# vstroebel/jpeg-encoder

Measured on NVIDIA B200. Metric: megapixels/sec encoded, byte-identical to the reference restatement, higher is better.
Workload: dtype u8 in / i32 arithmetic / i16 coefficients

## Files before the change

jpeg_encoder_b200/csrc/api.cu:

```cuda
#include <cuda_runtime.h>

#include <cstdio>
#include <cstdlib>
#include <algorithm>
#include <cstring>
#include <string>
#include <condition_variable>
#include <mutex>
#include <thread>
#include <vector>

#include "../../include/jpegenc_b200.h"
#include "copy_pool.h"
#include "host.h"
#include "kernels.h"

using namespace jpgb;

namespace {

bool poison_alloc() {
    const char *e = std::getenv("JPGB_POISON_ALLOC");
    return e && e[0] == '1';
}

struct DevBuf {
    void *p = nullptr;
    size_t cap = 0;
    cudaError_t reserve(size_t bytes) {
        if (bytes <= cap) return cudaSuccess;
        if (p) cudaFree(p);
        p = nullptr;
        cap = 0;
        size_t want = bytes + bytes / 8 + 256;
        want = (want + 255) & ~(size_t)255;
        cudaError_t e = cudaMalloc(&p, want);
        if (e == cudaSuccess) cap = want;
        if (e == cudaSuccess && poison_alloc()) {
            e = cudaMemset(p, 0xFF, want);
            if (e == cudaSuccess) e = cudaDeviceSynchronize();
        }
        return e;
    }
    template <typename T>
    T *as() const { return static_cast<T *>(p); }
    void release() {
        if (p) cudaFree(p);
        p = nullptr;
        cap = 0;
    }
};

struct PinnedBuf {
    void *p = nullptr;
    size_t cap = 0;
    cudaError_t reserve(size_t bytes) {
        if (bytes <= cap) return cudaSuccess;
        if (p) cudaFreeHost(p);
        p = nullptr;
        cap = 0;
        const size_t want = bytes + bytes / 8 + 256;
        cudaError_t e = cudaMallocHost(&p, want);
        if (e == cudaSuccess) {
            cap = want;
            if (poison_alloc()) std::memset(p, 0xFF, want);
        }
        return e;
    }
    template <typename T>
    T *as() const { return static_cast<T *>(p); }
    void release() {
        if (p) cudaFreeHost(p);
        p = nullptr;
        cap = 0;
    }
};

}

namespace {
struct PlanSig {
    jpgb_params p;
    jpgb_strip strip;
    uint32_t is_strip, planar;
};
inline PlanSig plan_sig(const Plan &plan) {
    PlanSig s;
    std::memset(&s, 0, sizeof(s));
    s.p.width = plan.p.width;
    s.p.height = plan.p.height;
    s.p.color_type = plan.p.color_type;
    s.p.quality = plan.p.quality;
    s.p.sampling = plan.p.sampling & 0x7F;
    for (int t = 0; t < 2; ++t) {
        s.p.qtable_kind[t] = plan.p.qtable_kind[t];
        if (plan.p.qtable_kind[t] == JPGB_QT_CUSTOM) std::memcpy(s.p.qtable_custom[t], plan.p.qtable_custom[t], sizeof(s.p.qtable_custom[t]));
    }
    s.p.progressive_scans = plan.p.progressive_scans;
    s.p.optimize_huffman = plan.p.optimize_huffman;
    s.p.restart_interval = plan.p.restart_interval;
    if (plan.is_strip) {
        s.strip.strip_index = plan.strip.strip_index;
        s.strip.n_strips = plan.strip.n_strips;
        s.strip.first_row = plan.strip.first_row;
        s.strip.rows = plan.strip.rows;
        s.strip.full_height = plan.strip.full_height;
    }
    s.is_strip = plan.is_strip;
    s.planar = plan.planar;
    return s;
}
struct CapKey {
    PlanSig sig;
    uint64_t raw_bytes;
    uint32_t n, pad;
};
struct GraphKey {
    EntropyBuffers b;
    CoderLaunch coder;
    PlanSig sig;
    uint64_t misc[8];
    uint32_t n, flags;
};
}

struct jpgb_encoder {
    int device = 0;
    cudaStream_t stream = nullptr;
    bool own_stream = false;
    std::string err;
    DevBuf pixels, coef, huff, hdr, hdr_len, scratch, pool, chunk_bits, chunk_pool, chunk_bitpos, seglen, segpos, ustream, ffcount, ffpos,
        out, scan_tmp, hist, piece_off, out2, pixels2, status, aux_status, hdr_parts;
    std::vector<uint8_t> last_tables;
    double ucap_ratio = 0;
    double pool_ratio = 0;
    PinnedBuf h_small, h_hist, h_tables, h_pieces, h_out, h_stage[2];
    cudaEvent_t ev_stage[2] = {};
    bool stage_busy[2] = {};
    CopyPool copy_pool;
    int out_slot = 0;
    cudaStream_t s_h2d = nullptr, s_d2h = nullptr;
    std::vector<cudaEvent_t> ev_slice;
    cudaEvent_t ev_in[2] = {}, ev_out[2] = {}, ev_enc[2] = {};
    bool timing = false;
    cudaEvent_t ev[JPGB_N_STAGES + 1][2] = {};
    bool ev_used[JPGB_N_STAGES] = {};
    float last_ms[JPGB_N_STAGES] = {};
    bool have_timing = false;
    uint32_t launches = 0;
    uint32_t last_piece_scans = 0;
    bool coef_tagged = false;
    PlanSig coef_sig{};
    const void *coef_pixels = nullptr;
    uint64_t coef_stride = 0;
    float coef_ms[2] = {0.f, 0.f};
    bool graphs_ok = true;
    struct CachedGraph {
        cudaGraphExec_t exec = nullptr;
        GraphKey key{};
        uint32_t launches = 0;
        uint64_t used = 0;
    } graphs[4];
    uint64_t graph_clock = 0;
    bool have_caps = false;
    CapKey cap_key{};
    uint64_t caps[3] = {};
    uint64_t out_total = 0;
};

namespace {

int fail(jpgb_encoder *e, int code, const std::string &msg) {
    if (e) e->err = msg;
    return code;
}
int fail_cuda(jpgb_encoder *e, cudaError_t ce, const char *what) {
    return fail(e, JPGB_ERR_CUDA, std::string(what) + ": " + cudaGetErrorString(ce));
}
#define CK(call, what)                                        \
    do {                                                      \
        cudaError_t ce__ = (call);                            \
        if (ce__ != cudaSuccess) return fail_cuda(enc, ce__, what); \
    } while (0)

struct StageTimer {
    jpgb_encoder *enc;
    int stage;
    StageTimer(jpgb_encoder *e, int s) : enc(e), stage(s) {
        if (enc->timing) {
            if (!enc->ev_used[stage]) cudaEventRecord(enc->ev[stage][0], enc->stream);
        }
    }
    ~StageTimer() {
        if (enc->timing) {
            cudaEventRecord(enc->ev[stage][1], enc->stream);
            enc->ev_used[stage] = true;
        }
    }
};

void timing_begin(jpgb_encoder *enc) {
    for (int i = 0; i < JPGB_N_STAGES; ++i) enc->ev_used[i] = false;
    enc->have_timing = false;
    enc->launches = 0;
}
void timing_end(jpgb_encoder *enc) {
    if (!enc->timing) return;
    cudaStreamSynchronize(enc->stream);
    for (int i = 0; i < JPGB_N_STAGES; ++i) {
        enc->last_ms[i] = 0.f;
        if (enc->ev_used[i]) cudaEventElapsedTime(&enc->last_ms[i], enc->ev[i][0], enc->ev[i][1]);
    }
    enc->have_timing = true;
}

int validate_and_plan(jpgb_encoder *enc, const jpgb_params *p, size_t len_each, Plan &plan) {
    if (!p) return fail(enc, JPGB_ERR_BAD_PARAMS, "null params");
    if (p->color_type > JPGB_YCCK) return fail(enc, JPGB_ERR_BAD_PARAMS, "bad color_type");
    const size_t required = (size_t)p->width * p->height * (size_t)bytes_per_pixel(p->color_type);
    if (len_each < required) {
        char m[128];
        snprintf(m, sizeof(m), "Image data too small for dimensions and color_type: %zu need at least %zu", len_each, required);
        return fail(enc, JPGB_ERR_BAD_IMAGE_DATA, m);
    }
    const int rc = plan.build(*p);
    if (rc != JPGB_OK) return fail(enc, rc, rc == JPGB_ERR_ZERO_DIMENSIONS ? "Image dimensions must be non zero" : "invalid parameters");
    return JPGB_OK;
}

int encode_device(jpgb_encoder *enc, const Plan &plan, const uint8_t *d_pixels, size_t image_stride, uint32_t n,
                  std::vector<uint64_t> &offsets, std::vector<uint64_t> *piece_offsets = nullptr, const uint32_t *given_hist = nullptr,
                  bool coef_ready = false) {
    cudaStream_t st = enc->stream;
    DevPlan hp;
    plan.fill_device_plan(hp);
    StageAParams ap;
    plan.fill_stage_a(ap);

    const uint64_t n_blocks = plan.blocks_per_image * n;
    const uint64_t n_segs = (uint64_t)plan.segs_per_image * n;

    CK(enc->coef.reserve(n_blocks * 128), "alloc coefficients");
    if (!coef_ready) enc->coef_tagged = false;
    if (!coef_ready) {
        StageTimer t(enc, 0);
        ap.pixels = d_pixels;
        ap.coef = enc->coef.as<int16_t>();
        ap.image_stride = image_stride;
        CK(launch_stage_a(ap, n, st), "stage A launch");
        enc->launches += 1;
    }

    unsigned long long *aux_status = nullptr, *scan_err = nullptr;

    const bool optimized = plan.p.optimize_huffman != 0;
    const uint32_t n_huff = optimized ? n : 1;
    HuffTable tables[4];
    default_huffman_tables(reinterpret_cast<HuffTable(*)[2]>(tables));
    size_t hdr_stride = 0;
    uint32_t opt_head_len = 0, opt_tail_len = 0;
    int opt_tables = 0;
    CK(enc->huff.reserve((size_t)n_huff * kHuffWordsPerImage * 4), "alloc huffman tables");
    CK(enc->hdr_len.reserve((size_t)n_huff * 4), "alloc header lengths");
    if (!optimized) {
        std::vector<uint8_t> h = plan.prefix;
        plan.frame_header(reinterpret_cast<const HuffTable(*)[2]>(tables), h);
        h.insert(h.end(), plan.scans[0].sos.begin(), plan.scans[0].sos.end());
        hdr_stride = (h.size() + 15) & ~(size_t)15;
        const size_t tab_bytes = kHuffWordsPerImage * 4, blob = tab_bytes + hdr_stride + 4;
        CK(enc->h_tables.reserve(blob), "alloc tables (host)");
        uint8_t *hb = enc->h_tables.as<uint8_t>();
        std::vector<uint8_t> fresh(blob, 0);
        for (int t = 0; t < 4; ++t)
            if (!tables[t].device_words(t & 1, reinterpret_cast<uint32_t *>(fresh.data() + (size_t)t * 1024)))
                return fail(enc, JPGB_ERR_HUFFMAN, "a Huffman code plus its value bits exceeds 31 bits");
        std::memcpy(fresh.data() + tab_bytes, h.data(), h.size());
        const uint32_t hl = (uint32_t)h.size();
        std::memcpy(fresh.data() + tab_bytes + hdr_stride, &hl, 4);
        CK(enc->hdr.reserve(hdr_stride), "alloc headers");
        if (enc->last_tables != fresh) {
            CK(cudaStreamSynchronize(enc->stream), "staging reuse sync");
            enc->last_tables = fresh;
            std::memcpy(hb, fresh.data(), blob);
            CK(cudaMemcpyAsync(enc->huff.p, hb, tab_bytes, cudaMemcpyHostToDevice, st), "upload huffman tables");
            CK(cudaMemcpyAsync(enc->hdr.p, hb + tab_bytes, hdr_stride, cudaMemcpyHostToDevice, st), "upload headers");
            CK(cudaMemcpyAsync(enc->hdr_len.p, hb + tab_bytes + hdr_stride, 4, cudaMemcpyHostToDevice, st), "upload header lengths");
        }
    } else {
        std::vector<uint8_t> with, without;
        {
            HuffTable empty[2][2];
            const uint8_t none[16] = {0};
            for (auto &row : empty)
                for (HuffTable &e : row) e.set(none, nullptr, 0);
            with = plan.prefix;
            plan.frame_header(empty, with);
        }
        const int n_tables = plan.ncomp >= 3 ? 2 : 1;
        size_t dht_at = plan.prefix.size();
        while (dht_at + 3 < with.size() && !(with[dht_at] == 0xFF && with[dht_at + 1] == 0xC4))
            dht_at += 2 + ((size_t)with[dht_at + 2] << 8 | with[dht_at + 3]);
        std::vector<uint8_t> head(with.begin(), with.begin() + dht_at);
        std::vector<uint8_t> tail(with.begin() + dht_at + (size_t)n_tables * 2 * 21, with.end());
        tail.insert(tail.end(), plan.scans[0].sos.begin(), plan.scans[0].sos.end());
        hdr_stride = (head.size() + (size_t)n_tables * 2 * (21 + 256) + tail.size() + 15) & ~(size_t)15;
        const size_t blob = head.size() + tail.size();
        CK(enc->h_tables.reserve(blob + 16), "alloc header parts (host)");
        CK(enc->hdr_parts.reserve(blob + 16), "alloc header parts");
        std::vector<uint8_t> fresh(head);
        fresh.insert(fresh.end(), tail.begin(), tail.end());
        fresh.push_back(0xA5);
        if (enc->last_tables != fresh) {
            CK(cudaStreamSynchronize(enc->stream), "staging reuse sync");
            enc->last_tables = fresh;
            std::memcpy(enc->h_tables.p, fresh.data(), blob);
            CK(cudaMemcpyAsync(enc->hdr_parts.p, enc->h_tables.p, blob, cudaMemcpyHostToDevice, st), "upload header parts");
        }
        const size_t hist_words = (size_t)n * 2 * 2 * 257;
        CK(enc->hist.reserve(hist_words * 4), "alloc histogram");
        if (given_hist) {
            CK(enc->h_hist.reserve(hist_words * 4), "alloc histogram (host)");
            CK(cudaStreamSynchronize(enc->stream), "staging reuse sync");
            std::memcpy(enc->h_hist.p, given_hist, hist_words * 4);
            CK(cudaMemcpyAsync(enc->hist.p, enc->h_hist.p, hist_words * 4, cudaMemcpyHostToDevice, st), "upload histogram");
        }
        CK(enc->hdr.reserve((size_t)n * hdr_stride), "alloc headers");
        opt_head_len = (uint32_t)head.size();
        opt_tail_len = (uint32_t)tail.size();
        opt_tables = n_tables;
    }
    auto enqueue_tables = [&]() -> int {
        StageTimer t(enc, 1);
        if (!given_hist) {
            CK(cudaMemsetAsync(enc->hist.p, 0, (size_t)n * 2 * 2 * 257 * 4, st), "clear histogram");
            CK(launch_histogram(hp, enc->coef.as<int16_t>(), n, enc->hist.as<uint32_t>(), st), "histogram launch");
            enc->launches += 1;
        }
        CK(launch_build_tables(enc->hist.as<uint32_t>(), 1, opt_tables, n, enc->huff.as<uint32_t>(), enc->hdr_parts.as<uint8_t>(), opt_head_len,
                               enc->hdr_parts.as<uint8_t>() + opt_head_len, opt_tail_len, enc->hdr.as<uint8_t>(), (uint32_t)hdr_stride,
                               enc->hdr_len.as<uint32_t>(), aux_status, st),
           "table build launch");
        enc->launches += 1;
        return JPGB_OK;
    };

    const uint64_t n_chunks = (uint64_t)plan.chunks_per_image * n;
    CK(enc->chunk_bits.reserve(n_chunks * 4), "alloc chunk sizes");
    CK(enc->chunk_pool.reserve(n_chunks * 4), "alloc chunk places");
    CK(enc->chunk_bitpos.reserve((n_chunks + 1) * 8), "alloc chunk positions");
    CK(enc->seglen.reserve(n_segs * 4), "alloc seglen");
    CK(enc->segpos.reserve((n_segs + 1) * 8), "alloc segpos");
    CoderLaunch coder{};
    CK(coder_launch_config(hp, n, coder), "coder configuration");
    CK(enc->scratch.reserve(coder.scratch_bytes), "alloc coder scratch");

    EntropyBuffers b{};
    b.coef = enc->coef.as<int16_t>();
    b.huff = enc->huff.as<uint32_t>();
    b.huff_per_image = optimized ? 1 : 0;
    b.scratch = enc->scratch.as<uint32_t>();
    b.chunk_bits = enc->chunk_bits.as<uint32_t>();
    b.chunk_pool = enc->chunk_pool.as<uint32_t>();
    b.chunk_bitpos = enc->chunk_bitpos.as<unsigned long long>();
    b.seglen = enc->seglen.as<uint32_t>();
    b.segpos = enc->segpos.as<unsigned long long>();
    b.hdr_len = enc->hdr_len.as<uint32_t>();
    b.hdr = enc->hdr.as<uint8_t>();
    b.hdr_stride = (uint32_t)hdr_stride;


    const uint64_t raw_bytes = (uint64_t)plan.p.width * plan.p.height * plan.bpp * n;
    uint64_t ucap = enc->ucap_ratio > 0 ? (uint64_t)(raw_bytes * enc->ucap_ratio) + (uint64_t)n * 4096 + 65536
                                        : raw_bytes / 3 + (uint64_t)n * 4096 + 65536;
    uint64_t ocap = ucap + ucap / 32 + 4096;
    uint64_t pool_units = (enc->pool_ratio > 0 ? (uint64_t)(raw_bytes * enc->pool_ratio) : raw_bytes / 3) / 16 + n_chunks + 4096;
    uint64_t ubytes = 0, total = 0, pool_used = 0;
    CK(enc->h_small.reserve((size_t)(2 * kStatusWords + n + 1) * 8), "alloc readback");
    b.n_segs_total = n_segs;
    CapKey ck;
    std::memset(&ck, 0, sizeof(ck));
    ck.sig = plan_sig(plan);
    ck.raw_bytes = raw_bytes;
    ck.n = n;
    if (enc->have_caps && std::memcmp(&enc->cap_key, &ck, sizeof(ck)) == 0) {
        ucap = enc->caps[0];
        ocap = enc->caps[1];
        pool_units = enc->caps[2];
    }
    if (const char *tight = std::getenv("JPGB_TIGHT_CAPS")) {
        const std::string t = std::string(",") + tight + ",";
        if (t.find(",pool,") != std::string::npos) pool_units = 1;
        if (t.find(",stream,") != std::string::npos) ucap = kStuffChunk;
        if (t.find(",out,") != std::string::npos) ocap = 4096;
    }
    bool coded = false;
    const char *poison_env = std::getenv("JPGB_POISON_STREAM");
    const bool poison = poison_env && poison_env[0] == '1';
    for (int attempt = 0;; ++attempt) {
        ucap = (ucap + kStuffChunk - 1) / kStuffChunk * kStuffChunk;
        const uint64_t n_pieces = ucap / kStuffChunk;
        CK(enc->ustream.reserve(ucap + 64), "alloc unstuffed stream");
        const size_t mask_bytes = (size_t)(ucap / 32 + 2) * 4;
        CK(enc->status.reserve((size_t)(n + 1 + 2 * kStatusWords) * 8 + mask_bytes), "alloc status and raw mask");
        CK(enc->ffcount.reserve((n_pieces + 1) * 4), "alloc ff counts");
        CK(enc->ffpos.reserve((n_pieces + 2) * 8), "alloc ff positions");
        CK(enc->scan_tmp.reserve(scan_tmp_bytes(std::max<uint64_t>(n_pieces, std::max(n_chunks, n_segs)))), "alloc scan scratch");
        CK(enc->pool.reserve(pool_units * 16), "alloc chunk pool");
        DevBuf &outb = enc->out_slot ? enc->out2 : enc->out;
        CK(outb.reserve(ocap + 64), "alloc output");
        if (piece_offsets) {
            CK(enc->piece_off.reserve((plan.scans.size() + 1) * 8), "alloc piece offsets");
            CK(enc->h_pieces.reserve((plan.scans.size() + 1) * 8), "alloc piece offsets (host)");
        }
        b.pool = enc->pool.as<uint32_t>();
        b.pool_cap = pool_units;
        b.ustream = enc->ustream.as<uint8_t>();
        b.file_off = enc->status.as<unsigned long long>();
        b.status = b.file_off + (n + 1);
        aux_status = b.status + kStatusWords;
        scan_err = b.status + 3;
        b.raw_mask = reinterpret_cast<uint32_t *>(b.status + 2 * kStatusWords);
        b.ffcount = enc->ffcount.as<uint32_t>();
        b.ffpos = enc->ffpos.as<unsigned long long>();
        b.scan_tmp = enc->scan_tmp.p;
        b.out = outb.as<uint8_t>();
        b.ustream_cap = ucap;
        b.out_cap = ocap;
        const bool with_tables = optimized && attempt == 0, with_coder = !coded;
        auto enqueue = [&]() -> int {
            if (with_coder) {
                CK(cudaMemsetAsync(b.status, 0, 2 * kStatusWords * 8 + mask_bytes, st), "clear status and raw mask");
            } else {
                CK(cudaMemsetAsync(b.status, 0, 4 * 8, st), "clear status");
                CK(cudaMemsetAsync(b.raw_mask, 0, mask_bytes, st), "clear raw mask");
            }
            if (with_tables) {
                const int rc = enqueue_tables();
                if (rc != JPGB_OK) return rc;
            }
            if (with_coder) {
                StageTimer t(enc, 2);
                CK(launch_encode_chunks(b, hp, n, coder, st), "coding launch");
                enc->launches += 1;
                const bool few_chunks = n_chunks <= 4096, few_segs = n_segs <= 4096;
                if (!few_chunks) CK(launch_exclusive_scan(b.chunk_bits, b.chunk_bitpos, n_chunks, b.scan_tmp, st, &enc->launches, scan_err), "chunk position scan");
                if (few_segs) {
                    CK(launch_positions(b, hp, n, few_chunks, st), "positions launch");
                    enc->launches += 1;
                } else {
                    if (few_chunks) CK(launch_exclusive_scan(b.chunk_bits, b.chunk_bitpos, n_chunks, b.scan_tmp, st, &enc->launches, scan_err), "chunk position scan");
                    CK(launch_segment_lengths(b, hp, n, st), "segment length launch");
                    CK(launch_exclusive_scan(b.seglen, b.segpos, n_segs, b.scan_tmp, st, &enc->launches, scan_err), "segment position scan");
                    enc->launches += 1;
                }
            }
            {
                StageTimer t(enc, 3);
                if (poison) CK(cudaMemsetAsync(b.ustream, 0xFF, ucap + 64, st), "poison stream");
                CK(launch_segment_leads(b, hp, n, st), "segment lead launch");
                CK(launch_place_chunks(b, hp, n, st), "placement launch");
                enc->launches += 2;
            }
            {
                StageTimer t(enc, 4);
                CK(launch_count_ff(b, st), "count ff launch");
                if (ff_scan_needed(b)) CK(launch_exclusive_scan(b.ffcount, b.ffpos, n_pieces, b.scan_tmp, st, &enc->launches, scan_err), "ff scan");
                CK(launch_stuff_scatter(b, hp, n, piece_offsets ? enc->piece_off.as<unsigned long long>() : nullptr, st), "scatter launch");
                enc->launches += 2;
                if (piece_offsets)
                    CK(cudaMemcpyAsync(enc->h_pieces.p, enc->piece_off.p, (plan.scans.size() + 1) * 8, cudaMemcpyDeviceToHost, st), "read piece offsets");
                CK(cudaMemcpyAsync(enc->h_small.p, b.file_off, (size_t)(n + 1 + 2 * kStatusWords) * 8, cudaMemcpyDeviceToHost, st), "read file offsets and status");
            }
            return JPGB_OK;
        };
        bool replayed = false;
        if (attempt == 0 && enc->graphs_ok && !enc->timing) {
            GraphKey gk;
            std::memset(&gk, 0, sizeof(gk));
            gk.b = b;
            gk.sig = ck.sig;
            gk.n = n;
            gk.coder = coder;
            gk.flags = (optimized ? 1u : 0u) | (piece_offsets ? 2u : 0u) | (given_hist ? 4u : 0u) | (poison ? 8u : 0u) | (uint32_t)hdr_stride << 8;
            gk.misc[0] = (uint64_t)enc->hist.p;
            gk.misc[1] = (uint64_t)enc->huff.p;
            gk.misc[2] = (uint64_t)enc->hdr_parts.p;
            gk.misc[3] = (uint64_t)enc->piece_off.p;
            gk.misc[4] = (uint64_t)enc->h_small.p;
            gk.misc[5] = (uint64_t)enc->h_pieces.p;
            gk.misc[6] = ((uint64_t)opt_head_len << 32) | opt_tail_len;
            gk.misc[7] = (uint64_t)enc->coef.p;
            jpgb_encoder::CachedGraph *slot = nullptr, *victim = &enc->graphs[0];
            for (auto &g : enc->graphs) {
                if (g.exec && std::memcmp(&gk, &g.key, sizeof(gk)) == 0) slot = &g;
                if (!g.exec || (victim->exec && g.used < victim->used)) victim = &g;
            }
            if (!slot) {
                if (victim->exec) cudaGraphExecDestroy(victim->exec), victim->exec = nullptr;
                const uint32_t launches_before = enc->launches;
                if (cudaStreamBeginCapture(st, cudaStreamCaptureModeThreadLocal) == cudaSuccess) {
                    const int rc = enqueue();
                    cudaGraph_t graph = nullptr;
                    const cudaError_t ce = cudaStreamEndCapture(st, &graph);
                    if (rc == JPGB_OK && ce == cudaSuccess && graph && cudaGraphInstantiate(&victim->exec, graph, 0) == cudaSuccess) {
                        victim->key = gk;
                        victim->launches = enc->launches - launches_before;
                        slot = victim;
                    } else {
                        victim->exec = nullptr;
                        enc->graphs_ok = false;
                    }
                    if (graph) cudaGraphDestroy(graph);
                    enc->launches = launches_before;
                    cudaGetLastError();
                } else {
                    enc->graphs_ok = false;
                    cudaGetLastError();
                }
            }
            if (slot) {
                slot->used = ++enc->graph_clock;
                CK(cudaGraphLaunch(slot->exec, st), "graph launch");
                enc->launches += slot->launches;
                replayed = true;
            }
        }
        if (!replayed) {
            const int rc = enqueue();
            if (rc != JPGB_OK) return rc;
        }
        CK(cudaStreamSynchronize(st), "final sync");
        const uint64_t *status = enc->h_small.as<uint64_t>() + (n + 1);
        if (status[3]) return fail(enc, JPGB_ERR_CUDA, "internal: prefix-sum look-back timed out");
        if (status[2] & 8) return fail(enc, JPGB_ERR_BAD_PARAMS, "a scan segment exceeds 4 GiB (use a restart interval)");
        if (with_tables && (status[kStatusWords + 2] & 16)) return fail(enc, JPGB_ERR_HUFFMAN, "an optimized Huffman code does not fit (longer than 32 bits, or code plus value bits beyond 31)");
        ubytes = status[0];
        if (with_coder) pool_used = status[5];
        if (status[2] == 0) {
            total = ubytes + status[1];
            break;
        }
        if (attempt >= 3) return fail(enc, JPGB_ERR_CUDA, "internal: buffer capacity retry did not converge");
        if (status[2] & 4) {
            pool_units = pool_used + pool_used / 64 + 4096;
            coded = false;
        } else {
            coded = true;
        }
        if (status[2] & 1) {
            ucap = ubytes + ubytes / 16 + 65536;
            ocap = ucap + ucap / 8 + 4096;
        } else if (status[2] & 2) {
            ocap = ubytes + status[1] + 4096;
        }
    }
    auto settle = [](uint64_t cap, uint64_t need, uint64_t slack) {
        const uint64_t lo = need + need / 20 + slack / 2, hi = need + need * 2 / 5 + 2 * slack;
        return (cap >= lo && cap <= hi) ? cap : need + need * 3 / 20 + slack;
    };
    enc->cap_key = ck;
    enc->caps[0] = settle(ucap, ubytes, (uint64_t)n * 4096 + 65536);
    enc->caps[1] = settle(ocap, total, 4096);
    enc->caps[1] = std::max(enc->caps[1], enc->caps[0] + enc->caps[0] / 64);
    enc->caps[2] = settle(pool_units, pool_used, 4096);
    enc->have_caps = true;
    enc->pool_ratio = std::max(enc->pool_ratio * 0.98, 1.1 * (double)((pool_used > n_chunks ? pool_used - n_chunks : 0) * 16) / (double)std::max<uint64_t>(raw_bytes, 1));
    enc->ucap_ratio = std::max(enc->ucap_ratio * 0.98, 1.15 * (double)ubytes / (double)std::max<uint64_t>(raw_bytes, 1));
    CK(cudaStreamSynchronize(st), "final sync");
    if (piece_offsets) {
        piece_offsets->assign(enc->h_pieces.as<uint64_t>(), enc->h_pieces.as<uint64_t>() + plan.scans.size() + 1);
        enc->last_piece_scans = (uint32_t)plan.scans.size();
    }
    offsets.assign(enc->h_small.as<uint64_t>(), enc->h_small.as<uint64_t>() + n + 1);
    enc->out_total = total;
    if (offsets[n] != total) return fail(enc, JPGB_ERR_CUDA, "internal: file offsets disagree with stream size");
    return JPGB_OK;
}

constexpr size_t kStageBytes = 16u << 20;
cudaError_t upload_host(jpgb_encoder *enc, void *d_dst, const uint8_t *src, size_t bytes, cudaStream_t s) {
    cudaPointerAttributes attr{};
    const bool pinned = cudaPointerGetAttributes(&attr, src) == cudaSuccess && (attr.type == cudaMemoryTypeHost || attr.type == cudaMemoryTypeManaged);
    cudaGetLastError();
    if (pinned || bytes <= 65536) return cudaMemcpyAsync(d_dst, src, bytes, cudaMemcpyHostToDevice, s);
    size_t piece = kStageBytes;
    if (bytes >= kStageBytes && bytes < 2 * kStageBytes) piece = ((bytes / 2 + (1u << 20) - 1) >> 20) << 20;
    unsigned hw = std::thread::hardware_concurrency();
    if (const char *e = std::getenv("JPGB_COPY_THREADS")) hw = (unsigned)std::max(1, std::atoi(e));
    for (size_t off = 0, k = 0; off < bytes; off += piece, ++k) {
        const int b = (int)(k & 1);
        const size_t n = std::min(piece, bytes - off);
        cudaError_t e = enc->h_stage[b].reserve(kStageBytes);
        if (e != cudaSuccess) return e;
        if (enc->stage_busy[b]) {
            e = cudaEventSynchronize(enc->ev_stage[b]);
            if (e != cudaSuccess) return e;
        }
        unsigned threads = (unsigned)std::min<size_t>(4, n >> 22);
        if (hw && threads > hw) threads = hw;
        enc->copy_pool.copy(enc->h_stage[b].p, src + off, n, threads);
        e = cudaMemcpyAsync(static_cast<uint8_t *>(d_dst) + off, enc->h_stage[b].p, n, cudaMemcpyHostToDevice, s);
        if (e != cudaSuccess) return e;
        e = cudaEventRecord(enc->ev_stage[b], s);
        if (e != cudaSuccess) return e;
        enc->stage_busy[b] = true;
    }
    return cudaSuccess;
}

int encode_host_pipelined(jpgb_encoder *enc, const Plan &plan, const uint8_t *const *pixels, uint32_t n,
                          std::vector<uint64_t> &offsets) {
    const size_t img_bytes = (size_t)plan.p.width * plan.p.height * plan.bpp;
    const size_t stride = (img_bytes + 255) & ~(size_t)255;
    uint32_t chunk = (uint32_t)std::max<size_t>(1, (96u << 20) / stride);
    chunk = std::min(chunk, n);
    const uint32_t n_chunks = (n + chunk - 1) / chunk;
    CK(enc->pixels.reserve(stride * chunk), "alloc pixels");
    if (n_chunks > 1) CK(enc->pixels2.reserve(stride * chunk), "alloc pixels");
    CK(enc->h_out.reserve(std::max<size_t>(img_bytes * n / 3, 1 << 20)), "alloc pinned output");
    offsets.assign(1, 0);
    cudaStream_t st = enc->stream;

    if (n == 1 && !plan.planar && img_bytes >= (48u << 20)) {
        const size_t row_bytes = (size_t)plan.p.width * plan.bpp;
        const uint32_t mcu_px = 8 * plan.vmax;
        uint32_t rows_per_slice = (uint32_t)std::max<size_t>(1, (32u << 20) / (row_bytes * mcu_px));
        rows_per_slice = (rows_per_slice + 3) & ~3u;
        const uint32_t n_slices = (plan.mcu_rows + rows_per_slice - 1) / rows_per_slice;
        CK(enc->pixels.reserve(stride), "alloc pixels");
        CK(enc->coef.reserve(plan.blocks_per_image * 128), "alloc coefficients");
        enc->coef_tagged = false;
        while (enc->ev_slice.size() < n_slices) {
            cudaEvent_t e;
            CK(cudaEventCreateWithFlags(&e, cudaEventDisableTiming), "create event");
            enc->ev_slice.push_back(e);
        }
        StageAParams ap;
        plan.fill_stage_a(ap);
        for (uint32_t k = 0; k < n_slices; ++k) {
            const size_t r0 = (size_t)k * rows_per_slice * mcu_px, r1 = std::min<size_t>(plan.p.height, r0 + (size_t)rows_per_slice * mcu_px);
            CK(upload_host(enc, enc->pixels.as<uint8_t>() + r0 * row_bytes, pixels[0] + r0 * row_bytes, (r1 - r0) * row_bytes, enc->s_h2d), "upload slice");
            CK(cudaEventRecord(enc->ev_slice[k], enc->s_h2d), "record slice");
        }
        for (uint32_t k = 0; k < n_slices; ++k) {
            const size_t r0 = (size_t)k * rows_per_slice * mcu_px, r1 = std::min<size_t>(plan.p.height, r0 + (size_t)rows_per_slice * mcu_px);
            StageAParams sp = ap;
            sp.pixels = enc->pixels.as<uint8_t>() + r0 * row_bytes;
            sp.coef = enc->coef.as<int16_t>();
            sp.image_stride = stride;
            sp.height = (int)(r1 - r0);
            sp.mcu_row0 = (int)(k * rows_per_slice);
            sp.mcu_rows = (int)std::min<uint32_t>(rows_per_slice, plan.mcu_rows - k * rows_per_slice);
            CK(cudaStreamWaitEvent(st, enc->ev_slice[k], 0), "wait slice");
            CK(launch_stage_a(sp, 1, st), "stage A launch");
            enc->launches += 1;
        }
        std::vector<uint64_t> off;
        const int rc = encode_device(enc, plan, enc->pixels.as<uint8_t>(), stride, 1, off, nullptr, nullptr, true);
        if (rc != JPGB_OK) return rc;
        CK(enc->h_out.reserve(std::max<size_t>(off[1], 1 << 20)), "alloc pinned output");
        CK(cudaMemcpyAsync(enc->h_out.p, enc->out.p, off[1], cudaMemcpyDeviceToHost, st), "download file");
        CK(cudaStreamSynchronize(st), "download sync");
        offsets.push_back(off[1]);
        return JPGB_OK;
    }

    auto upload = [&](uint32_t c) -> cudaError_t {
        DevBuf &px = (c & 1) ? enc->pixels2 : enc->pixels;
        const uint32_t lo = c * chunk, hi = std::min(n, lo + chunk);
        if (c >= 2) {
            cudaError_t e = cudaStreamWaitEvent(enc->s_h2d, enc->ev_enc[c & 1], 0);
            if (e != cudaSuccess) return e;
        }
        for (uint32_t i = lo; i < hi; ++i) {
            cudaError_t e = upload_host(enc, px.as<uint8_t>() + stride * (i - lo), pixels[i], img_bytes, enc->s_h2d);
            if (e != cudaSuccess) return e;
        }
        return cudaEventRecord(enc->ev_in[c & 1], enc->s_h2d);
    };

    {
        StageTimer t(enc, 5);
        CK(upload(0), "upload pixels");
    }
    uint64_t total = 0;
    for (uint32_t c = 0; c < n_chunks; ++c) {
        const uint32_t lo = c * chunk, hi = std::min(n, lo + chunk), cn = hi - lo;
        if (c + 1 < n_chunks) CK(upload(c + 1), "upload pixels");
        DevBuf &px = (c & 1) ? enc->pixels2 : enc->pixels;
        CK(cudaStreamWaitEvent(st, enc->ev_in[c & 1], 0), "wait upload");
        if (c >= 2) CK(cudaStreamWaitEvent(st, enc->ev_out[c & 1], 0), "wait download");
        enc->out_slot = (int)(c & 1);
        std::vector<uint64_t> off;
        const uint32_t launches_before = enc->launches;
        const int rc = encode_device(enc, plan, px.as<uint8_t>(), stride, cn, off);
        enc->out_slot = 0;
        if (rc != JPGB_OK) return rc;
        (void)launches_before;
        CK(cudaEventRecord(enc->ev_enc[c & 1], st), "record encode");
        const uint64_t bytes = off[cn];
        if (total + bytes > enc->h_out.cap) {
            CK(cudaStreamSynchronize(enc->s_d2h), "download sync");
            PinnedBuf bigger;
            CK(bigger.reserve((total + bytes) * 2), "grow pinned output");
            std::memcpy(bigger.p, enc->h_out.p, total);
            enc->h_out.release();
            enc->h_out = bigger;
        }
        DevBuf &ob = (c & 1) ? enc->out2 : enc->out;
        CK(cudaMemcpyAsync(enc->h_out.as<uint8_t>() + total, ob.p, bytes, cudaMemcpyDeviceToHost, enc->s_d2h), "download files");
        CK(cudaEventRecord(enc->ev_out[c & 1], enc->s_d2h), "record download");
        for (uint32_t i = 0; i < cn; ++i) offsets.push_back(total + off[i + 1]);
        total += bytes;
    }
    {
        StageTimer t(enc, 6);
        CK(cudaStreamSynchronize(enc->s_d2h), "download sync");
    }
    return JPGB_OK;
}

int encode_host_batch(jpgb_encoder *enc, const jpgb_params *p, const uint8_t *const *pixels, size_t len_each, uint32_t n,
                      uint8_t **outs, size_t *out_lens, const uint8_t **pinned_base, uint64_t *pinned_offsets) {
    if (!enc) return JPGB_ERR_BAD_PARAMS;
    const bool pinned_api = pinned_base != nullptr;
    if (!pixels || n == 0 || (pinned_api ? !pinned_offsets : (!outs || !out_lens))) return fail(enc, JPGB_ERR_BAD_PARAMS, "null argument");
    if (!pinned_api)
        for (uint32_t i = 0; i < n; ++i) outs[i] = nullptr, out_lens[i] = 0;
    Plan plan;
    int rc = validate_and_plan(enc, p, len_each, plan);
    if (rc != JPGB_OK) return rc;
    CK(cudaSetDevice(enc->device), "cudaSetDevice");
    const bool was_timing = enc->timing;
    enc->timing = false;
    timing_begin(enc);
    std::vector<uint64_t> off;
    rc = encode_host_pipelined(enc, plan, pixels, n, off);
    enc->timing = was_timing;
    if (rc != JPGB_OK) return rc;
    if (pinned_api) {
        *pinned_base = enc->h_out.as<uint8_t>();
        std::memcpy(pinned_offsets, off.data(), (size_t)(n + 1) * 8);
        return JPGB_OK;
    }
    for (uint32_t i = 0; i < n; ++i) {
        const size_t sz = (size_t)(off[i + 1] - off[i]);
        outs[i] = static_cast<uint8_t *>(std::malloc(sz ? sz : 1));
        if (!outs[i]) {
            for (uint32_t k = 0; k < i; ++k) std::free(outs[k]), outs[k] = nullptr;
            return fail(enc, JPGB_ERR_NOMEM, "out of host memory");
        }
        out_lens[i] = sz;
        std::memcpy(outs[i], enc->h_out.as<uint8_t>() + off[i], sz);
    }
    return JPGB_OK;
}

}

extern "C" {

void jpgb_params_default(jpgb_params *p, uint8_t quality) {
    std::memset(p, 0, sizeof(*p));
    p->quality = quality;
    p->sampling = quality < 90 ? 0x22 : 0x11;
    p->density_unit = 0;
    p->density_x = p->density_y = 1;
}

int jpgb_encoder_create(int device, void *cuda_stream, jpgb_encoder **out) {
    if (!out) return JPGB_ERR_BAD_PARAMS;
    *out = nullptr;
    int count = 0;
    if (cudaGetDeviceCount(&count) != cudaSuccess || device < 0 || device >= count) return JPGB_ERR_CUDA;
    cudaDeviceProp prop;
    if (cudaGetDeviceProperties(&prop, device) != cudaSuccess) return JPGB_ERR_CUDA;
    if (prop.major != 10) return JPGB_ERR_CUDA;
    if (cudaSetDevice(device) != cudaSuccess) return JPGB_ERR_CUDA;
    jpgb_encoder *e = new (std::nothrow) jpgb_encoder();
    if (!e) return JPGB_ERR_NOMEM;
    e->device = device;
    if (cuda_stream) {
        e->stream = static_cast<cudaStream_t>(cuda_stream);
    } else {
        if (cudaStreamCreateWithFlags(&e->stream, cudaStreamNonBlocking) != cudaSuccess) {
            delete e;
            return JPGB_ERR_CUDA;
        }
        e->own_stream = true;
    }
    for (int i = 0; i < JPGB_N_STAGES; ++i)
        for (int k = 0; k < 2; ++k) cudaEventCreate(&e->ev[i][k]);
    cudaStreamCreateWithFlags(&e->s_h2d, cudaStreamNonBlocking);
    cudaStreamCreateWithFlags(&e->s_d2h, cudaStreamNonBlocking);
    for (int i = 0; i < 2; ++i) {
        cudaEventCreateWithFlags(&e->ev_in[i], cudaEventDisableTiming);
        cudaEventCreateWithFlags(&e->ev_out[i], cudaEventDisableTiming);
        cudaEventCreateWithFlags(&e->ev_enc[i], cudaEventDisableTiming);
        cudaEventCreateWithFlags(&e->ev_stage[i], cudaEventDisableTiming);
    }
    *out = e;
    return JPGB_OK;
}

void jpgb_encoder_destroy(jpgb_encoder *e) {
    if (!e) return;
    cudaSetDevice(e->device);
    cudaStreamSynchronize(e->stream);
    DevBuf *bufs[] = {&e->pixels, &e->coef, &e->huff, &e->hdr, &e->hdr_len, &e->scratch, &e->pool, &e->chunk_bits, &e->chunk_pool, &e->chunk_bitpos, &e->seglen, &e->segpos,
                      &e->ustream, &e->ffcount, &e->ffpos, &e->out, &e->scan_tmp, &e->hist, &e->piece_off, &e->out2, &e->pixels2, &e->status, &e->aux_status, &e->hdr_parts};
    for (DevBuf *b : bufs) b->release();
    e->h_small.release();
    e->h_hist.release();
    e->h_tables.release();
    e->h_pieces.release();
    e->h_out.release();
    for (auto &g : e->graphs)
        if (g.exec) cudaGraphExecDestroy(g.exec);
    if (e->s_h2d) cudaStreamDestroy(e->s_h2d);
    if (e->s_d2h) cudaStreamDestroy(e->s_d2h);
    for (cudaEvent_t ev : e->ev_slice) cudaEventDestroy(ev);
    for (int i = 0; i < 2; ++i) {
        if (e->ev_in[i]) cudaEventDestroy(e->ev_in[i]);
        if (e->ev_out[i]) cudaEventDestroy(e->ev_out[i]);
        if (e->ev_enc[i]) cudaEventDestroy(e->ev_enc[i]);
        if (e->ev_stage[i]) cudaEventDestroy(e->ev_stage[i]);
        e->h_stage[i].release();
    }
    for (int i = 0; i < JPGB_N_STAGES; ++i)
        for (int k = 0; k < 2; ++k)
            if (e->ev[i][k]) cudaEventDestroy(e->ev[i][k]);
    if (e->own_stream) cudaStreamDestroy(e->stream);
    delete e;
}

const char *jpgb_last_error(const jpgb_encoder *e) { return e ? e->err.c_str() : "no encoder"; }

int jpgb_encode(jpgb_encoder *enc, const jpgb_params *p, const uint8_t *pixels, size_t len, uint8_t **out, size_t *out_len) {
    if (!out || !out_len) return JPGB_ERR_BAD_PARAMS;
    *out = nullptr;
    *out_len = 0;
    const uint8_t *px[1] = {pixels};
    return encode_host_batch(enc, p, px, len, 1, out, out_len, nullptr, nullptr);
}

void jpgb_free(void *buf) { std::free(buf); }

static int encode_planar_pinned(jpgb_encoder *enc, const jpgb_params *p, const uint8_t *const planes[4], size_t plane_len, size_t *out_len) {
    if (!p || !planes) return fail(enc, JPGB_ERR_BAD_PARAMS, "null argument");
    const uint8_t ct = p->color_type;
    if (ct != JPGB_LUMA && ct != JPGB_YCBCR && ct != JPGB_CMYK && ct != JPGB_YCCK)
        return fail(enc, JPGB_ERR_BAD_PARAMS, "planar input takes a JPEG colour type: Luma, Ycbcr, Cmyk or Ycck");
    const size_t plane_bytes = (size_t)p->width * p->height;
    if (plane_len < plane_bytes) return fail(enc, JPGB_ERR_BAD_IMAGE_DATA, "plane shorter than width*height");
    Plan plan;
    plan.planar = true;
    const int rc = plan.build(*p);
    if (rc != JPGB_OK) return fail(enc, rc, rc == JPGB_ERR_ZERO_DIMENSIONS ? "Image dimensions must be non zero" : "invalid parameters");
    CK(cudaSetDevice(enc->device), "cudaSetDevice");
    timing_begin(enc);
    const size_t stride = (plane_bytes * plan.ncomp + 255) & ~(size_t)255;
    CK(enc->pixels.reserve(stride), "alloc planes");
    for (int c = 0; c < plan.ncomp; ++c) {
        if (!planes[c]) return fail(enc, JPGB_ERR_BAD_PARAMS, "null plane");
        CK(upload_host(enc, enc->pixels.as<uint8_t>() + plane_bytes * c, planes[c], plane_bytes, enc->stream), "upload plane");
    }
    std::vector<uint64_t> off;
    const int rc2 = encode_device(enc, plan, enc->pixels.as<uint8_t>(), stride, 1, off);
    if (rc2 != JPGB_OK) return rc2;
    const size_t sz = (size_t)off[1];
    CK(enc->h_out.reserve(sz ? sz : 1), "alloc pinned output");
    CK(cudaMemcpyAsync(enc->h_out.p, enc->out.p, sz, cudaMemcpyDeviceToHost, enc->stream), "download file");
    CK(cudaStreamSynchronize(enc->stream), "download sync");
    *out_len = sz;
    timing_end(enc);
    return JPGB_OK;
}

int jpgb_encode_planar(jpgb_encoder *enc, const jpgb_params *p, const uint8_t *const planes[4], size_t plane_len, uint8_t **out,
                       size_t *out_len) {
    if (!enc) return JPGB_ERR_BAD_PARAMS;
    if (!out || !out_len) return fail(enc, JPGB_ERR_BAD_PARAMS, "null argument");
    *out = nullptr;
    *out_len = 0;
    size_t sz = 0;
    const int rc = encode_planar_pinned(enc, p, planes, plane_len, &sz);
    if (rc != JPGB_OK) return rc;
    *out = static_cast<uint8_t *>(std::malloc(sz ? sz : 1));
    if (!*out) return fail(enc, JPGB_ERR_NOMEM, "out of host memory");
    std::memcpy(*out, enc->h_out.p, sz);
    *out_len = sz;
    return JPGB_OK;
}

int jpgb_encode_planar_to_sink(jpgb_encoder *enc, const jpgb_params *p, const uint8_t *const planes[4], size_t plane_len,
                               jpgb_write_all_fn write_all, void *user) {
    if (!enc) return JPGB_ERR_BAD_PARAMS;
    if (!write_all) return fail(enc, JPGB_ERR_BAD_PARAMS, "null sink");
    size_t sz = 0;
    const int rc = encode_planar_pinned(enc, p, planes, plane_len, &sz);
    if (rc != JPGB_OK) return rc;
    if (write_all(user, enc->h_out.as<uint8_t>(), sz) != 0) return fail(enc, JPGB_ERR_SINK, "sink write_all failed");
    return JPGB_OK;
}

int jpgb_encode_to_sink(jpgb_encoder *enc, const jpgb_params *p, const uint8_t *pixels, size_t len, jpgb_write_all_fn write_all,
                        void *user) {
    if (!enc) return JPGB_ERR_BAD_PARAMS;
    if (!write_all) return fail(enc, JPGB_ERR_BAD_PARAMS, "null sink");
    const uint8_t *px[1] = {pixels};
    const uint8_t *files = nullptr;
    uint64_t offs[2] = {0, 0};
    const int rc = encode_host_batch(enc, p, px, len, 1, nullptr, nullptr, &files, offs);
    if (rc != JPGB_OK) return rc;
    if (write_all(user, files + offs[0], (size_t)(offs[1] - offs[0])) != 0) return fail(enc, JPGB_ERR_SINK, "sink write_all failed");
    return JPGB_OK;
}

int jpgb_encode_batch(jpgb_encoder *enc, const jpgb_params *p, const uint8_t *const *pixels, size_t len_each, uint32_t n,
                      uint8_t **outs, size_t *out_lens) {
    return encode_host_batch(enc, p, pixels, len_each, n, outs, out_lens, nullptr, nullptr);
}

int jpgb_encode_batch_pinned(jpgb_encoder *enc, const jpgb_params *p, const uint8_t *const *pixels, size_t len_each, uint32_t n,
                             const uint8_t **files, uint64_t *offsets) {
    if (!files) return JPGB_ERR_BAD_PARAMS;
    return encode_host_batch(enc, p, pixels, len_each, n, nullptr, nullptr, files, offsets);
}

int jpgb_encode_batch_device(jpgb_encoder *enc, const jpgb_params *p, const void *d_pixels, size_t image_stride, uint32_t n,
                             const void **d_files, uint64_t *offsets) {
    if (!enc) return JPGB_ERR_BAD_PARAMS;
    if (!d_pixels || !d_files || !offsets || n == 0) return fail(enc, JPGB_ERR_BAD_PARAMS, "null argument");
    Plan plan;
    int rc = validate_and_plan(enc, p, image_stride, plan);
    if (rc != JPGB_OK) return rc;
    CK(cudaSetDevice(enc->device), "cudaSetDevice");
    timing_begin(enc);
    std::vector<uint64_t> off;
    rc = encode_device(enc, plan, static_cast<const uint8_t *>(d_pixels), image_stride, n, off);
    if (rc != JPGB_OK) return rc;
    timing_end(enc);
    std::memcpy(offsets, off.data(), (size_t)(n + 1) * 8);
    *d_files = enc->out.p;
    return JPGB_OK;
}

int jpgb_scan_count(const jpgb_params *p, uint32_t *n_scans) {
    if (!p || !n_scans) return JPGB_ERR_BAD_PARAMS;
    Plan plan;
    const int rc = plan.build(*p);
    if (rc != JPGB_OK) return rc;
    *n_scans = (uint32_t)plan.scans.size();
    return JPGB_OK;
}

int jpgb_plan_strips(const jpgb_params *p, uint32_t max_strips, jpgb_strip *strips, uint32_t *n_strips) {
    if (!p || !strips || !n_strips || max_strips == 0) return JPGB_ERR_BAD_PARAMS;
    Plan plan;
    const int rc = plan.build(*p);
    if (rc != JPGB_OK) return rc;
    const uint32_t R = p->restart_interval;
    if (R == 0) return JPGB_ERR_BAD_PARAMS;
    auto gcd = [](uint64_t a, uint64_t b) { while (b) { const uint64_t t = a % b; a = b; b = t; } return a; };
    uint64_t step = 1;
    for (const Scan &s : plan.scans) {
        const uint64_t upr = s.comp < 0 ? plan.mcu_cols : (uint64_t)plan.comps[s.comp].v * plan.true_w[s.comp];
        const uint64_t need = R / gcd(R, upr);
        step = step / gcd(step, need) * need;
    }
    const uint64_t groups = (plan.mcu_rows + step - 1) / step;
    uint32_t n = (uint32_t)std::min<uint64_t>(max_strips, groups);
    if (n == 0) n = 1;
    const uint32_t rows_per_mcu = 8 * plan.vmax;
    uint64_t g0 = 0;
    for (uint32_t i = 0; i < n; ++i) {
        const uint64_t g1 = groups * (i + 1) / n;
        const uint64_t r0 = g0 * step * rows_per_mcu, r1 = std::min<uint64_t>(g1 * step * rows_per_mcu, p->height);
        strips[i].strip_index = i;
        strips[i].n_strips = n;
        strips[i].first_row = (uint16_t)r0;
        strips[i].rows = (uint16_t)(r1 - r0);
        strips[i].full_height = p->height;
        g0 = g1;
    }
    *n_strips = n;
    return JPGB_OK;
}

static int encode_strip(jpgb_encoder *enc, const jpgb_params *p, const jpgb_strip *strip, const void *d_pixels, const uint32_t *hist_total,
                        const void **d_bytes, uint64_t *piece_offsets) {
    if (!enc) return JPGB_ERR_BAD_PARAMS;
    if (!p || !strip || !d_pixels || !d_bytes || !piece_offsets) return fail(enc, JPGB_ERR_BAD_PARAMS, "null argument");
    if (p->color_type > JPGB_YCCK) return fail(enc, JPGB_ERR_BAD_PARAMS, "bad color_type");
    if ((p->optimize_huffman != 0) != (hist_total != nullptr))
        return fail(enc, JPGB_ERR_BAD_PARAMS, "optimized tables with strips take the whole image's histogram (jpgb_encode_strip_device_optimized); other settings take none");
    Plan plan;
    const int rc = plan.build(*p, strip);
    if (rc != JPGB_OK) return fail(enc, rc, "settings or strip geometry do not allow strip encoding (needs restart intervals aligned in every scan)");
    CK(cudaSetDevice(enc->device), "cudaSetDevice");
    timing_begin(enc);
    std::vector<uint64_t> off, pieces;
    const size_t stride = (size_t)p->width * strip->rows * bytes_per_pixel(p->color_type);
    bool reuse = false;
    if (hist_total && enc->coef_tagged && enc->coef_pixels == d_pixels && enc->coef_stride == uint64_t(stride)) {
        const PlanSig sig = plan_sig(plan);
        reuse = std::memcmp(&sig, &enc->coef_sig, sizeof(sig)) == 0;
    }
    const int rc2 = encode_device(enc, plan, static_cast<const uint8_t *>(d_pixels), stride, 1, off, &pieces, hist_total, reuse);
    enc->coef_tagged = false;
    if (rc2 != JPGB_OK) return rc2;
    timing_end(enc);
    if (reuse && enc->timing) {
        enc->last_ms[0] += enc->coef_ms[0];
        enc->last_ms[1] += enc->coef_ms[1];
    }
    std::memcpy(piece_offsets, pieces.data(), pieces.size() * 8);
    *d_bytes = enc->out.p;
    return JPGB_OK;
}

int jpgb_encode_strip_device(jpgb_encoder *enc, const jpgb_params *p, const jpgb_strip *strip, const void *d_pixels,
                             const void **d_bytes, uint64_t *piece_offsets) {
    return encode_strip(enc, p, strip, d_pixels, nullptr, d_bytes, piece_offsets);
}

int jpgb_encode_strip_device_optimized(jpgb_encoder *enc, const jpgb_params *p, const jpgb_strip *strip, const void *d_pixels,
                                       const uint32_t hist_total[JPGB_HIST_WORDS], const void **d_bytes, uint64_t *piece_offsets) {
    if (enc && !hist_total) return fail(enc, JPGB_ERR_BAD_PARAMS, "null histogram");
    return encode_strip(enc, p, strip, d_pixels, hist_total, d_bytes, piece_offsets);
}

int jpgb_strip_histogram_device(jpgb_encoder *enc, const jpgb_params *p, const jpgb_strip *strip, const void *d_pixels,
                                uint32_t hist[JPGB_HIST_WORDS], int16_t edge_dc[8]) {
    if (!enc) return JPGB_ERR_BAD_PARAMS;
    if (!p || !strip || !d_pixels || !hist || !edge_dc) return fail(enc, JPGB_ERR_BAD_PARAMS, "null argument");
    if (p->color_type > JPGB_YCCK || !p->optimize_huffman) return fail(enc, JPGB_ERR_BAD_PARAMS, "strip histograms belong to optimized Huffman tables");
    Plan plan;
    const int rc = plan.build(*p, strip);
    if (rc != JPGB_OK) return fail(enc, rc, "settings or strip geometry do not allow strip encoding (needs restart intervals aligned in every scan)");
    CK(cudaSetDevice(enc->device), "cudaSetDevice");
    cudaStream_t st = enc->stream;
    DevPlan hp;
    plan.fill_device_plan(hp);
    StageAParams ap;
    plan.fill_stage_a(ap);
    CK(enc->coef.reserve(plan.blocks_per_image * 128), "alloc coefficients");
    ap.pixels = static_cast<const uint8_t *>(d_pixels);
    ap.coef = enc->coef.as<int16_t>();
    ap.image_stride = (size_t)p->width * strip->rows * bytes_per_pixel(p->color_type);
    timing_begin(enc);
    {
        StageTimer t(enc, 0);
        CK(launch_stage_a(ap, 1, st), "stage A launch");
    }
    const size_t hist_bytes = JPGB_HIST_WORDS * 4;
    CK(enc->hist.reserve(hist_bytes), "alloc histogram");
    CK(enc->h_hist.reserve(hist_bytes + 16), "alloc histogram (host)");
    {
        StageTimer t(enc, 1);
        CK(cudaMemsetAsync(enc->hist.p, 0, hist_bytes, st), "clear histogram");
        CK(launch_histogram(hp, enc->coef.as<int16_t>(), 1, enc->hist.as<uint32_t>(), st), "histogram launch");
    }
    enc->launches = 2;
    CK(cudaMemcpyAsync(enc->h_hist.p, enc->hist.p, hist_bytes, cudaMemcpyDeviceToHost, st), "download histogram");
    int16_t *edge = reinterpret_cast<int16_t *>(enc->h_hist.as<uint8_t>() + hist_bytes);
    std::memset(edge, 0, 16);
    for (int c = 0; c < plan.ncomp; ++c) {
        const uint64_t first = plan.block_off[c], last = plan.block_off[c] + (uint64_t)plan.true_w[c] * plan.true_h[c] - 1;
        CK(cudaMemcpyAsync(edge + c, enc->coef.as<int16_t>() + first * 64, 2, cudaMemcpyDeviceToHost, st), "read edge DC");
        CK(cudaMemcpyAsync(edge + 4 + c, enc->coef.as<int16_t>() + last * 64, 2, cudaMemcpyDeviceToHost, st), "read edge DC");
    }
    CK(cudaStreamSynchronize(st), "histogram sync");
    std::memcpy(hist, enc->h_hist.p, hist_bytes);
    std::memcpy(edge_dc, edge, 16);
    enc->coef_sig = plan_sig(plan);
    enc->coef_pixels = d_pixels;
    enc->coef_stride = uint64_t(ap.image_stride);
    enc->coef_tagged = true;
    timing_end(enc);
    enc->coef_ms[0] = enc->timing ? enc->last_ms[0] : 0.f;
    enc->coef_ms[1] = enc->timing ? enc->last_ms[1] : 0.f;
    return JPGB_OK;
}

int jpgb_merge_strip_histograms(const jpgb_params *p, uint32_t n_strips, const uint32_t hist_sum[JPGB_HIST_WORDS], const int16_t *edge_dc,
                                uint32_t hist_total[JPGB_HIST_WORDS]) {
    if (!p || !hist_sum || !edge_dc || !hist_total || n_strips == 0) return JPGB_ERR_BAD_PARAMS;
    Plan plan;
    const int rc = plan.build(*p);
    if (rc != JPGB_OK) return rc;
    std::memcpy(hist_total, hist_sum, JPGB_HIST_WORDS * 4);
    auto category = [](int diff) {
        int a = (int16_t)diff;
        a = a < 0 ? -a : a;
        int n = 0;
        while (a) ++n, a >>= 1;
        return n;
    };
    for (uint32_t s = 1; s < n_strips; ++s)
        for (int c = 0; c < plan.ncomp; ++c) {
            uint32_t *dc = hist_total + (size_t)plan.comps[c].dc_table * 2 * 257;
            const int first = edge_dc[s * 8 + c], prev_last = edge_dc[(s - 1) * 8 + 4 + c];
            dc[category(first)] -= 1;
            dc[category(first - prev_last)] += 1;
        }
    return JPGB_OK;
}

int jpgb_gather_target_create(jpgb_encoder *enc, size_t capacity, void **d_target, uint8_t ipc_handle[64]) {
    if (!enc) return JPGB_ERR_BAD_PARAMS;
    if (!d_target || !ipc_handle || capacity == 0) return fail(enc, JPGB_ERR_BAD_PARAMS, "null argument");
    static_assert(sizeof(cudaIpcMemHandle_t) == 64, "the C ABI carries the IPC handle as 64 bytes");
    CK(cudaSetDevice(enc->device), "cudaSetDevice");
    void *p = nullptr;
    CK(cudaMalloc(&p, capacity + 64), "alloc gather target");
    cudaIpcMemHandle_t h;
    const cudaError_t ce = cudaIpcGetMemHandle(&h, p);
    if (ce != cudaSuccess) {
        cudaFree(p);
        return fail_cuda(enc, ce, "cudaIpcGetMemHandle");
    }
    std::memcpy(ipc_handle, &h, 64);
    *d_target = p;
    return JPGB_OK;
}

int jpgb_gather_target_open(jpgb_encoder *enc, const uint8_t ipc_handle[64], void **d_target) {
    if (!enc) return JPGB_ERR_BAD_PARAMS;
    if (!d_target || !ipc_handle) return fail(enc, JPGB_ERR_BAD_PARAMS, "null argument");
    CK(cudaSetDevice(enc->device), "cudaSetDevice");
    cudaIpcMemHandle_t h;
    std::memcpy(&h, ipc_handle, 64);
    void *p = nullptr;
    CK(cudaIpcOpenMemHandle(&p, h, cudaIpcMemLazyEnablePeerAccess), "cudaIpcOpenMemHandle (peer access over NVLink)");
    *d_target = p;
    return JPGB_OK;
}

int jpgb_gather_target_close(jpgb_encoder *enc, void *d_target, int opened_from_handle) {
    if (!enc) return JPGB_ERR_BAD_PARAMS;
    if (!d_target) return JPGB_OK;
    CK(cudaSetDevice(enc->device), "cudaSetDevice");
    CK(cudaStreamSynchronize(enc->stream), "sync before releasing the gather target");
    if (opened_from_handle) CK(cudaIpcCloseMemHandle(d_target), "cudaIpcCloseMemHandle");
    else CK(cudaFree(d_target), "free gather target");
    return JPGB_OK;
}

int jpgb_last_piece_offsets_device(jpgb_encoder *enc, const uint64_t **d_offsets, uint32_t *n_scans) {
    if (!enc) return JPGB_ERR_BAD_PARAMS;
    if (!d_offsets || !n_scans || !enc->piece_off.p || enc->last_piece_scans == 0) return fail(enc, JPGB_ERR_BAD_PARAMS, "no strip has been encoded on this context");
    *d_offsets = enc->piece_off.as<uint64_t>();
    *n_scans = enc->last_piece_scans;
    return JPGB_OK;
}

int jpgb_gather_place_pieces(jpgb_encoder *enc, void *d_target, size_t target_capacity, const uint64_t *d_table, uint32_t world, uint32_t rank,
                             uint64_t *d_total) {
    if (!enc) return JPGB_ERR_BAD_PARAMS;
    if (!d_target || !d_table || world == 0 || rank >= world || enc->last_piece_scans == 0) return fail(enc, JPGB_ERR_BAD_PARAMS, "bad gather arguments");
    CK(cudaSetDevice(enc->device), "cudaSetDevice");
    CK(enc->aux_status.reserve(kStatusWords * 8), "alloc status");
    CK(launch_place_pieces(enc->out.as<uint8_t>(), static_cast<uint8_t *>(d_target), target_capacity, reinterpret_cast<const unsigned long long *>(d_table),
                           world, rank, enc->last_piece_scans, reinterpret_cast<unsigned long long *>(d_total),
                           enc->aux_status.as<unsigned long long>() + 4, enc->stream),
       "piece placement launch");
    return JPGB_OK;
}

int jpgb_download(jpgb_encoder *enc, const void *d_src, size_t n, void *host_dst) {
    if (!enc) return JPGB_ERR_BAD_PARAMS;
    if (n == 0) return JPGB_OK;
    if (!d_src || !host_dst) return fail(enc, JPGB_ERR_BAD_PARAMS, "null argument");
    CK(cudaSetDevice(enc->device), "cudaSetDevice");
    CK(cudaMemcpyAsync(host_dst, d_src, n, cudaMemcpyDeviceToHost, enc->stream), "download");
    CK(cudaStreamSynchronize(enc->stream), "download sync");
    return JPGB_OK;
}

int jpgb_coef_layout_for(const jpgb_params *p, jpgb_coef_layout *l) {
    if (!p || !l) return JPGB_ERR_BAD_PARAMS;
    Plan plan;
    const int rc = plan.build(*p);
    if (rc != JPGB_OK) return rc;
    std::memset(l, 0, sizeof(*l));
    l->n_components = (uint32_t)plan.ncomp;
    for (int c = 0; c < plan.ncomp; ++c) {
        l->blocks_w[c] = plan.pad_w[c];
        l->blocks_h[c] = plan.pad_h[c];
        l->true_w[c] = plan.true_w[c];
        l->true_h[c] = plan.true_h[c];
        l->block_offset[c] = plan.block_off[c];
        l->slot_base[c] = plan.slot_base[c];
        l->comp_h[c] = plan.comps[c].h;
        l->comp_v[c] = plan.comps[c].v;
    }
    l->blocks_per_image = plan.blocks_per_image;
    l->mcu_order = plan.mode == Mode::Interleaved;
    l->mcu_cols = plan.mcu_cols;
    l->mcu_rows = plan.mcu_rows;
    l->blocks_per_mcu = plan.bpu_interleaved;
    return JPGB_OK;
}

int jpgb_stage_a_device(jpgb_encoder *enc, const jpgb_params *p, const void *d_pixels, size_t image_stride, uint32_t n, void *d_coef) {
    if (!enc) return JPGB_ERR_BAD_PARAMS;
    if (!d_pixels || !d_coef || n == 0) return fail(enc, JPGB_ERR_BAD_PARAMS, "null argument");
    Plan plan;
    const int rc = validate_and_plan(enc, p, image_stride, plan);
    if (rc != JPGB_OK) return rc;
    CK(cudaSetDevice(enc->device), "cudaSetDevice");
    StageAParams ap;
    plan.fill_stage_a(ap);
    ap.pixels = static_cast<const uint8_t *>(d_pixels);
    ap.coef = static_cast<int16_t *>(d_coef);
    ap.image_stride = image_stride;
    enc->launches = 0;
    CK(launch_stage_a(ap, n, enc->stream), "stage A launch");
    enc->launches = 1;
    return JPGB_OK;
}

void jpgb_encoder_set_timing(jpgb_encoder *enc, int enabled) {
    if (enc) enc->timing = enabled != 0;
}
int jpgb_encoder_last_timing(const jpgb_encoder *enc, float ms[JPGB_N_STAGES]) {
    if (!enc || !enc->have_timing) return JPGB_ERR_BAD_PARAMS;
    std::memcpy(ms, enc->last_ms, sizeof(enc->last_ms));
    return JPGB_OK;
}
uint32_t jpgb_encoder_last_launch_count(const jpgb_encoder *enc) { return enc ? enc->launches : 0; }

int jpgb_build_header(const jpgb_params *p, uint8_t *buf, size_t cap, size_t *len) {
    if (!p || !len) return JPGB_ERR_BAD_PARAMS;
    Plan plan;
    const int rc = plan.build(*p);
    if (rc != JPGB_OK) return rc;
    HuffTable huff[2][2];
    default_huffman_tables(huff);
    std::vector<uint8_t> h = plan.prefix;
    plan.frame_header(huff, h);
    h.insert(h.end(), plan.scans[0].sos.begin(), plan.scans[0].sos.end());
    *len = h.size();
    if (buf) std::memcpy(buf, h.data(), std::min(cap, h.size()));
    return JPGB_OK;
}

int jpgb_optimized_huffman_table(const uint32_t freq[257], uint8_t length[16], uint8_t values[256], uint32_t *n_values) {
    if (!freq || !length || !values || !n_values) return JPGB_ERR_BAD_PARAMS;
    HuffTable t;
    if (!t.set_optimized(freq)) return JPGB_ERR_HUFFMAN;
    std::memcpy(length, t.length, 16);
    std::memcpy(values, t.values.data(), t.values.size());
    *n_values = (uint32_t)t.values.size();
    return JPGB_OK;
}

int jpgb_optimized_huffman_tables_device(jpgb_encoder *enc, const uint32_t *freq, uint32_t n, int ac, uint8_t *lengths, uint8_t *values,
                                         uint32_t *n_values, uint32_t *words, int *status) {
    if (!enc) return JPGB_ERR_BAD_PARAMS;
    if (!freq || !lengths || !values || !n_values || !words || !status || n == 0) return fail(enc, JPGB_ERR_BAD_PARAMS, "null argument");
    CK(cudaSetDevice(enc->device), "cudaSetDevice");
    cudaStream_t st = enc->stream;
    DevBuf d_hist, d_words, d_dht, d_len, d_bad;
    auto release = [&] { d_hist.release(); d_words.release(); d_dht.release(); d_len.release(); d_bad.release(); };
    std::vector<uint8_t> dht((size_t)n * 277);
    std::vector<uint32_t> len(n), bad(n);
    cudaError_t e = d_hist.reserve((size_t)n * 257 * 4);
    if (e == cudaSuccess) e = d_words.reserve((size_t)n * 1024);
    if (e == cudaSuccess) e = d_dht.reserve((size_t)n * 277);
    if (e == cudaSuccess) e = d_len.reserve((size_t)n * 4);
    if (e == cudaSuccess) e = d_bad.reserve((size_t)n * 4);
    if (e == cudaSuccess) e = cudaMemcpyAsync(d_hist.p, freq, (size_t)n * 257 * 4, cudaMemcpyHostToDevice, st);
    if (e == cudaSuccess) e = launch_build_single_tables(d_hist.as<uint32_t>(), n, ac, d_words.as<uint32_t>(), d_dht.as<uint8_t>(), d_len.as<uint32_t>(), d_bad.as<uint32_t>(), st);
    if (e == cudaSuccess) e = cudaMemcpyAsync(words, d_words.p, (size_t)n * 1024, cudaMemcpyDeviceToHost, st);
    if (e == cudaSuccess) e = cudaMemcpyAsync(dht.data(), d_dht.p, dht.size(), cudaMemcpyDeviceToHost, st);
    if (e == cudaSuccess) e = cudaMemcpyAsync(len.data(), d_len.p, (size_t)n * 4, cudaMemcpyDeviceToHost, st);
    if (e == cudaSuccess) e = cudaMemcpyAsync(bad.data(), d_bad.p, (size_t)n * 4, cudaMemcpyDeviceToHost, st);
    if (e == cudaSuccess) e = cudaStreamSynchronize(st);
    release();
    if (e != cudaSuccess) return fail_cuda(enc, e, "device table build");
    for (uint32_t i = 0; i < n; ++i) {
        status[i] = bad[i] ? JPGB_ERR_HUFFMAN : JPGB_OK;
        n_values[i] = bad[i] ? 0 : len[i] - 21;
        std::memcpy(lengths + (size_t)i * 16, dht.data() + (size_t)i * 277 + 5, 16);
        std::memcpy(values + (size_t)i * 256, dht.data() + (size_t)i * 277 + 21, 256);
    }
    return JPGB_OK;
}

const char *jpgb_version(void) { return "jpeg-encoder_b200 0.1 (sm_100a; parity target: jpeg-encoder 0.7.0)"; }

}
```

jpeg_encoder_b200/csrc/entropy.cu:

```cuda
#include <mutex>

#include "kernels.h"

namespace jpgb {
namespace {

__device__ __forceinline__ int find_scan_by_seg(const DevPlan &P, unsigned s) {
    int lo = 0, hi = P.n_scans - 1;
    while (lo < hi) {
        const int mid = (lo + hi + 1) >> 1;
        if (P.scans[mid].seg_base <= s) lo = mid;
        else hi = mid - 1;
    }
    return lo;
}
__device__ __forceinline__ int find_scan_by_chunk(const DevPlan &P, unsigned c) {
    int lo = 0, hi = P.n_scans - 1;
    while (lo < hi) {
        const int mid = (lo + hi + 1) >> 1;
        if (P.scans[mid].chunk_base <= c) lo = mid;
        else hi = mid - 1;
    }
    return lo;
}

__device__ __forceinline__ void value_code(int v, int &size, uint32_t &bits) {
    const int a = v < 0 ? -v : v;
    int top;
    asm("bfind.u32 %0, %1;" : "=r"(top) : "r"(a));
    size = top + 1;
    uint32_t mask;
    asm("bmsk.clamp.b32 %0, 0, %1;" : "=r"(mask) : "r"(size));
    bits = (uint32_t)(v + (v >> 31)) & mask;
}

__device__ __forceinline__ unsigned nonzero16x2(unsigned x) {
    unsigned r;
    asm("min.u16x2 %0, %1, %2;" : "=r"(r) : "r"(x), "r"(0x00010001u));
    return r;
}

template <int T>
struct BitSink {
    unsigned long long acc = 0;
    int n = 0;
    unsigned off = 0;
    uint32_t *slot0;

    __device__ __forceinline__ BitSink(uint32_t *scratch, int visit) : slot0(scratch + visit) {}
    __device__ __forceinline__ void put(uint32_t code, int len) {
        acc = (acc << len) | code;
        n += len;
        if (n >= 32) {
            n -= 32;
            *reinterpret_cast<uint32_t *>(reinterpret_cast<char *>(slot0) + off) = (uint32_t)(acc >> n);
            off += T * 4;
        }
    }
    __device__ __forceinline__ unsigned finish() {
        if (n > 0) *reinterpret_cast<uint32_t *>(reinterpret_cast<char *>(slot0) + off) = (uint32_t)(acc << (32 - n));
        return off / (T * 4) * 32 + n;
    }
};

constexpr uint32_t kCodeBits = 0x07FFFFFFu;

constexpr int kStageStride = 72;
constexpr int kAsmWordsProg = 3072;

__device__ __forceinline__ unsigned long long zrl_markers(unsigned long long m, int first_ac) {
    const unsigned long long z = m | (1ull << (first_ac - 1));
    unsigned long long s = z;
    s |= s << 1;
    s |= s << 2;
    s |= s << 4;
    const unsigned long long s16 = s | (s << 8);
    const unsigned long long s32 = s16 | (s16 << 16);
    const unsigned long long s48 = s32 | (s16 << 32);
    unsigned long long marks = ((z << 16) & ~s16) | ((z << 32) & ~s32) | ((z << 48) & ~s48);
    const int top = 63 - __clzll((long long)m);
    marks &= top > 0 ? (~0ull >> (64 - top)) : 0ull;
    return marks;
}

template <int BASE, int T>
__device__ __forceinline__ void code_half(unsigned m, int &next, unsigned c_shared, const uint32_t *__restrict__ tab, BitSink<T> &sink) {
#pragma unroll 1
    while (m) {
        int p;
        asm("bfind.u32 %0, %1;" : "=r"(p) : "r"(m));
        unsigned bit;
        asm("bmsk.clamp.b32 %0, %1, 1;" : "=r"(bit) : "r"(p));
        m ^= bit;
        const int k = BASE + 31 - p;
        int v;
        asm("ld.shared.s16 %0, [%1];" : "=r"(v) : "r"(c_shared + 2 * k));
        const int run = k - next;
        next = k + 1;
        int size;
        uint32_t bits;
        value_code(v, size, bits);
        const uint32_t e = (tab + run * 16)[size];
        sink.put((e & kCodeBits) | bits, (int)(e >> 27));
    }
}
template <int T>
__device__ __forceinline__ void code_nonzeros(unsigned lo_rev, unsigned hi_rev, int first_ac, int se, const int16_t *__restrict__ c,
                                              const uint32_t *__restrict__ tab, BitSink<T> &sink) {
    int next = first_ac;
    const unsigned c_shared = (unsigned)__cvta_generic_to_shared(c);
    code_half<0, T>(lo_rev, next, c_shared, tab, sink);
    code_half<32, T>(hi_rev, next, c_shared, tab, sink);
    if (next <= se) {
        const uint32_t e = tab[0];
        sink.put(e & kCodeBits, (int)(e >> 27));
    }
}

struct __align__(16) ItemInfo {
    unsigned long long img, blk0, chunk_index0;
    unsigned v_in_seg0, n_valid, group;
    int done;
};

template <int T, bool FULL>
struct CoderSmem {
    static constexpr int kCoefBytes = T * kStageStride * 2;
    static constexpr int kAsmWords = FULL ? kCoefBytes / 4 : kAsmWordsProg;
    static constexpr int oAsm = FULL ? 0 : kCoefBytes;
    static constexpr int oAc = kCoefBytes + (FULL ? 0 : kAsmWordsProg * 4);
    static constexpr int oDc = oAc + 2048;
    static constexpr int oSlot = oDc + 256;
    static constexpr int oBin = oSlot + 128;
    static constexpr int oNb = oBin + 256;
    static constexpr int oOrder = oNb + T * 4;
    static constexpr int oWsum = oOrder + T * 2;
    static constexpr int oItem = oWsum + 64;
    static constexpr int kBytes = oItem + 2 * 64;
};

__host__ __device__ constexpr int coder_min_ctas(int T, bool full) { return full && T >= 128 ? 1280 / T : 1024 / T; }

template <int T, bool FULL>
__global__ void __launch_bounds__(T, coder_min_ctas(T, FULL)) encode_chunks_kernel(const __grid_constant__ EntropyBuffers b, const __grid_constant__ DevPlan P,
                                                          unsigned long long n_items) {
    using L = CoderSmem<T, FULL>;
    extern __shared__ __align__(16) unsigned char smem[];
    int16_t *coef = reinterpret_cast<int16_t *>(smem);
    uint32_t *asmbuf = reinterpret_cast<uint32_t *>(smem + L::oAsm);
    uint32_t *ac_tab = reinterpret_cast<uint32_t *>(smem + L::oAc);
    uint2 *dc_tab = reinterpret_cast<uint2 *>(smem + L::oDc);
    uint32_t *slot_tab = reinterpret_cast<uint32_t *>(smem + L::oSlot);
    uint32_t *bin = reinterpret_cast<uint32_t *>(smem + L::oBin);
    uint32_t *nbv = reinterpret_cast<uint32_t *>(smem + L::oNb);
    auto visit_meta = [&](int v) { return reinterpret_cast<uint4 *>(smem + v * (kStageStride * 2) + 128); };
    uint16_t *order = reinterpret_cast<uint16_t *>(smem + L::oOrder);
    uint32_t *wsum = reinterpret_cast<uint32_t *>(smem + L::oWsum);
    ItemInfo *items = reinterpret_cast<ItemInfo *>(smem + L::oItem);

    const int tid = threadIdx.x, lane = tid & 31, warp = tid >> 5;
    uint32_t *scratch = b.scratch + (size_t)blockIdx.x * (T * kSlotWords);
    long long tab_img = -1;
    for (int i = tid; i < 64; i += T) bin[i] = 0;
    if (tid < kMaxSlots) slot_tab[tid] = (unsigned)P.comp_tbl[P.slot_comp[tid]] | (unsigned)P.slot_back[tid] << 8 | (unsigned)P.slot_first[tid] << 16;
    auto decode = [&](unsigned long long ticket, ItemInfo &it) {
        it.done = ticket >= n_items;
        if (it.done) return;
        unsigned long long img;
        unsigned r;
        if ((ticket >> 32) == 0) {
            unsigned q;
            divmod((unsigned)ticket, P.div_items, q, r);
            img = q;
        } else {
            img = ticket / P.items_per_image;
            r = (unsigned)(ticket - img * P.items_per_image);
        }
        int g = 0;
        while (g + 1 < P.n_groups && r >= P.groups[g + 1].item_base) ++g;
        const DevGroup &G = P.groups[g];
        unsigned seg, chunk;
        divmod(r - G.item_base, G.div_cps, seg, chunk);
        const unsigned long long seg_start = (unsigned long long)seg * G.seg_visits;
        const unsigned long long v0 = seg_start + (unsigned long long)chunk * T;
        unsigned long long seg_end = seg_start + G.seg_visits;
        if (seg_end > G.n_visits) seg_end = G.n_visits;
        it.img = img;
        it.group = (unsigned)g;
        it.v_in_seg0 = chunk * T;
        it.n_valid = v0 < seg_end ? (unsigned)(seg_end - v0 < (unsigned long long)T ? seg_end - v0 : T) : 0u;
        it.blk0 = img * P.blocks_per_image + G.block_base + v0;
        it.chunk_index0 = img * P.chunks_per_image + (r - G.item_base);
    };
    unsigned long long next_ticket = 0;
    if (tid == 0) {
        decode(atomicAdd(b.status + 4, 1ull), items[0]);
        next_ticket = atomicAdd(b.status + 4, 1ull);
    }

    for (unsigned round = 0;; ++round) {
        __syncthreads();
        const ItemInfo it = items[round & 1];
        if (it.done) break;
        if (tid == 0) {
            decode(next_ticket, items[(round & 1) ^ 1]);
            next_ticket = atomicAdd(b.status + 4, 1ull);
        }
        if (it.n_valid == 0) {
            for (int j = tid; j < P.spg; j += T) {
                const unsigned long long ci = it.chunk_index0 + P.scans[it.group + j * P.n_groups].chunk_base;
                b.chunk_bits[ci] = 0;
                b.chunk_pool[ci] = 0;
            }
            continue;
        }
        const DevGroup &G = P.groups[it.group];
        const bool valid = (unsigned)tid < it.n_valid;

        const long long want_tab = b.huff_per_image ? (long long)it.img : 0;
        if (want_tab != tab_img) {
            const uint32_t *set = b.huff + (size_t)want_tab * kHuffWordsPerImage;
            for (int i = tid; i < 512; i += T) {
                ac_tab[i] = __ldg(set + (i >> 8) * 512 + 256 + (i & 255));
            }
            if (tid < 32) {
                const uint32_t e = __ldg(set + (tid >> 4) * 512 + (tid & 15));
                dc_tab[tid] = make_uint2(e & kCodeBits, e >> 27);
            }
            tab_img = want_tab;
        }

        const int16_t *src_blocks = b.coef + it.blk0 * 64;
        {
            const unsigned pieces = it.n_valid * 8;
            const char *g = reinterpret_cast<const char *>(src_blocks) + (size_t)tid * 16;
            const unsigned d = (unsigned)__cvta_generic_to_shared(coef) + (tid >> 3) * (kStageStride * 2) + (tid & 7) * 16;
            if (it.n_valid == T) {
#pragma unroll
                for (int k = 0; k < 8; ++k)
                    asm volatile("cp.async.cg.shared.global [%0], [%1], 16;" ::"r"(d + k * (T / 8) * (kStageStride * 2)), "l"(g + k * T * 16) : "memory");
            } else {
#pragma unroll
                for (int k = 0; k < 8; ++k)
                    if ((unsigned)(tid + k * T) < pieces)
                        asm volatile("cp.async.cg.shared.global [%0], [%1], 16;" ::"r"(d + k * (T / 8) * (kStageStride * 2)), "l"(g + k * T * 16) : "memory");
            }
            asm volatile("cp.async.wait_all;" ::: "memory");
        }
        __syncthreads();

        unsigned long long m_all = 0;
        int dcdiff = 0, tbl = 0;
        if (valid) {
            const uint4 *mine = reinterpret_cast<const uint4 *>(coef + tid * kStageStride);
            unsigned m_lo = 0, m_hi = 0;
#pragma unroll
            for (int w = 0; w < 8; ++w) {
                const uint4 q = mine[w];
                unsigned byte = __dp2a_lo(nonzero16x2(q.x), 0x0201u, 0u);
                byte = __dp2a_lo(nonzero16x2(q.y), 0x0804u, byte);
                byte = __dp2a_lo(nonzero16x2(q.z), 0x2010u, byte);
                byte = __dp2a_lo(nonzero16x2(q.w), 0x8040u, byte);
                if (w < 4) m_lo |= byte << (8 * w);
                else m_hi |= byte << (8 * (w - 4));
            }
            m_all = (((unsigned long long)m_hi << 32) | m_lo) & ~1ull;
            const unsigned v_in_seg = it.v_in_seg0 + tid;
            unsigned unit = v_in_seg, slot = 0;
            if (G.bpu > 1) divmod(v_in_seg, G.div_bpu, unit, slot);
            const unsigned sinfo = G.comp < 0 ? slot_tab[slot] : ((unsigned)P.comp_tbl[G.comp] | 0x10100u);
            tbl = sinfo & 0xFF;
            const int back = (sinfo >> 8) & 0xFF;
            const bool first_of_comp = (sinfo >> 16) != 0;
            int prev = 0;
            if (!(unit == 0 && first_of_comp)) prev = tid >= back ? (int)coef[(tid - back) * kStageStride] : (int)__ldg(src_blocks + ((long long)tid - back) * 64);
            dcdiff = (int)(int16_t)(coef[tid * kStageStride] - prev);
        }

        for (int j = 0; j < (FULL ? 1 : P.spg); ++j) {
            const DevScan &S = P.scans[it.group + j * P.n_groups];
            const int ss = FULL ? 0 : S.ss, se = FULL ? 63 : S.se;
            const int first_ac = ss == 0 ? 1 : ss;
            unsigned m_lo = 0, m_hi = 0;
            uint32_t first = 0;
            if (valid) {
                if (se > 0) {
                    unsigned long long m = FULL ? m_all : m_all & (~0ull << first_ac) & (~0ull >> (63 - se));
                    m |= zrl_markers(m, first_ac);
                    m_lo = __brev((unsigned)m);
                    m_hi = __brev((unsigned)(m >> 32));
                }
                if (ss == 0) {
                    int size;
                    uint32_t bits;
                    value_code(dcdiff, size, bits);
                    const uint2 e = dc_tab[tbl * 16 + size];
                    first = e.x | bits | e.y << 27;
                }
            }
            *visit_meta(tid) = make_uint4(m_lo, m_hi, first, (unsigned)tbl | (valid ? 0x100u : 0u));
            if (se > 0) {
                const int nnz = __popc(m_lo) + __popc(m_hi);
                const unsigned rank = atomicAdd(&bin[nnz], 1u);
                __syncthreads();
                {
                    const unsigned a = bin[2 * lane], c = bin[2 * lane + 1];
                    unsigned inc = a + c;
#pragma unroll
                    for (int d = 1; d < 32; d <<= 1) {
                        const unsigned o = __shfl_up_sync(0xffffffffu, inc, d);
                        if (lane >= d) inc += o;
                    }
                    const unsigned even = inc - a - c, odd = inc - c;
                    const unsigned e = __shfl_sync(0xffffffffu, even, nnz >> 1), o = __shfl_sync(0xffffffffu, odd, nnz >> 1);
                    order[((nnz & 1) ? o : e) + rank] = (uint16_t)tid;
                }
                __syncthreads();
                for (int i = tid; i < 64; i += T) bin[i] = 0;
            } else {
                order[tid] = (uint16_t)tid;
                __syncthreads();
            }

            if (j == 0) {
                const ItemInfo &nx = items[(round & 1) ^ 1];
                if (!nx.done && (unsigned)tid < nx.n_valid)
                    asm volatile("prefetch.global.L2 [%0];" ::"l"(b.coef + (nx.blk0 + tid) * 64));
            }
            {
                const int src = order[tid];
                const uint4 meta = *visit_meta(src);
                const unsigned inf = meta.w;
                unsigned nb = 0;
                if (inf & 0x100u) {
                    const uint32_t dc_code = meta.z;
                    BitSink<T> sink(scratch, src);
                    sink.put(dc_code & kCodeBits, (int)(dc_code >> 27));
                    if (se > 0) code_nonzeros<T>(meta.x, meta.y, first_ac, se, coef + src * kStageStride, ac_tab + (inf & 0xFF) * 256, sink);
                    nb = sink.finish();
                }
                nbv[src] = nb;
            }
            __syncthreads();

            const unsigned myb = nbv[tid];
            const unsigned nw = (myb + 31) >> 5;
            const uint32_t *mine = scratch + tid;
            uint32_t pre[4];
#pragma unroll
            for (int q = 0; q < 4; ++q) pre[q] = __ldcg(mine + q * T);
            unsigned inc = myb;
#pragma unroll
            for (int d = 1; d < 32; d <<= 1) {
                const unsigned o = __shfl_up_sync(0xffffffffu, inc, d);
                if (lane >= d) inc += o;
            }
            unsigned off = inc - myb, total = 0;
#pragma unroll
            for (int w = 0; w < T / 32; ++w) {
                const unsigned sw = __reduce_add_sync(0xffffffffu, nbv[w * 32 + lane]);
                if (w < warp) off += sw;
                total += sw;
            }
            const unsigned total_words = (total + 31) >> 5;
            const unsigned long long ci = it.chunk_index0 + S.chunk_base;
            const unsigned pool_units = (total_words + 3) >> 2;
            unsigned long long pool_at = 0;
            if (tid == 0) {
                if (pool_units) pool_at = atomicAdd(b.status + 5, (unsigned long long)pool_units);
                b.chunk_bits[ci] = total;
            }
            for (unsigned wb = 0; wb < total_words; wb += L::kAsmWords) {
                const unsigned nwin = total_words - wb < (unsigned)L::kAsmWords ? total_words - wb : (unsigned)L::kAsmWords;
                for (unsigned i = tid * 4; i < nwin; i += T * 4) *reinterpret_cast<uint4 *>(asmbuf + i) = make_uint4(0, 0, 0, 0);
                __syncthreads();
                if (myb) {
                    const unsigned d0 = off >> 5, dl = (off + myb - 1) >> 5, sft = off & 31;
                    auto word = [&](unsigned q) -> uint32_t {
                        if (q >= nw) return 0u;
                        if (q < 4) return q == 0 ? pre[0] : (q == 1 ? pre[1] : (q == 2 ? pre[2] : pre[3]));
                        return __ldcg(mine + q * T);
                    };
                    if (wb == 0 && dl < nwin) {
                        uint32_t prev = pre[0];
                        atomicOr(asmbuf + d0, prev >> sft);
                        unsigned jw = 1;
                        for (unsigned d = d0 + 1; d < dl; ++d, ++jw) {
                            const uint32_t cur = word(jw);
                            asmbuf[d] = __funnelshift_r(cur, prev, sft);
                            prev = cur;
                        }
                        if (dl > d0) atomicOr(asmbuf + dl, __funnelshift_r(word(jw), prev, sft));
                    } else {
                        const unsigned lo = d0 > wb ? d0 : wb, hi = dl < wb + nwin - 1 ? dl : wb + nwin - 1;
                        if (lo <= hi) {
                            unsigned jw = lo - d0;
                            uint32_t prev = jw > 0 ? word(jw - 1) : 0u;
                            for (unsigned d = lo; d <= hi; ++d, ++jw) {
                                const uint32_t cur = word(jw);
                                atomicOr(asmbuf + (d - wb), __funnelshift_r(cur, prev, sft));
                                prev = cur;
                            }
                        }
                    }
                }
                if (tid == 0 && wb == 0) {
                    if (pool_at + pool_units > b.pool_cap) {
                        atomicOr(b.status + 2, 4ull);
                        pool_at = ~0ull;
                    }
                    wsum[8] = (uint32_t)pool_at;
                    wsum[9] = (uint32_t)(pool_at >> 32);
                    b.chunk_pool[ci] = (uint32_t)pool_at;
                }
                __syncthreads();
                const unsigned long long at = ((unsigned long long)wsum[9] << 32) | wsum[8];
                if (at != ~0ull) {
                    uint4 *dst = reinterpret_cast<uint4 *>(b.pool) + at + (wb >> 2);
                    for (unsigned i = tid; i * 4 < nwin; i += T) dst[i] = reinterpret_cast<const uint4 *>(asmbuf)[i];
                }
                if (wb + L::kAsmWords < total_words || !FULL) __syncthreads();
            }
        }
    }
}

__device__ __forceinline__ unsigned lead_len(const EntropyBuffers &b, const DevPlan &P, unsigned long long img, int k,
                                             unsigned seg_in_scan) {
    if (P.scans[k].rst_base + seg_in_scan > 0) return 2;
    if (k > 0) return P.scans[k].sos_len;
    return b.hdr_len[b.huff_per_image ? img : 0];
}

__global__ void __launch_bounds__(256) segment_len_kernel(const __grid_constant__ EntropyBuffers b, const __grid_constant__ DevPlan P, unsigned long long n_segs) {
    const unsigned long long g = (unsigned long long)blockIdx.x * blockDim.x + threadIdx.x;
    if (g >= n_segs) return;
    const unsigned long long img = g / P.segs_per_image;
    const unsigned s = (unsigned)(g - img * P.segs_per_image);
    const int k = find_scan_by_seg(P, s);
    const DevScan &S = P.scans[k];
    const unsigned i = s - S.seg_base;
    const unsigned cps = P.groups[k % P.n_groups].cps;
    const unsigned long long c0 = img * P.chunks_per_image + S.chunk_base + (unsigned long long)i * cps;
    const unsigned long long bits = b.chunk_bitpos[c0 + cps] - b.chunk_bitpos[c0];
    const unsigned tail = (s == P.segs_per_image - 1 && P.has_eoi) ? 2u : 0u;
    const unsigned long long bytes = lead_len(b, P, img, k, i) + ((bits + 7) >> 3) + tail;
    if (bytes > 0xFFFFFFFFull) atomicOr(b.status + 2, 8ull);
    b.seglen[g] = (unsigned)bytes;
}

__device__ __forceinline__ unsigned long long segment_bytes(const EntropyBuffers &b, const DevPlan &P, unsigned long long g) {
    const unsigned long long img = g / P.segs_per_image;
    const unsigned s = (unsigned)(g - img * P.segs_per_image);
    const int k = find_scan_by_seg(P, s);
    const DevScan &S = P.scans[k];
    const unsigned i = s - S.seg_base;
    const unsigned cps = P.groups[k % P.n_groups].cps;
    const unsigned long long c0 = img * P.chunks_per_image + S.chunk_base + (unsigned long long)i * cps;
    const unsigned long long bits = b.chunk_bitpos[c0 + cps] - b.chunk_bitpos[c0];
    const unsigned tail = (s == P.segs_per_image - 1 && P.has_eoi) ? 2u : 0u;
    return lead_len(b, P, img, k, i) + ((bits + 7) >> 3) + tail;
}

__device__ __forceinline__ unsigned long long cta1024_exclusive(unsigned long long v, unsigned long long *sm, unsigned long long &total) {
    const int lane = threadIdx.x & 31, warp = threadIdx.x >> 5;
    unsigned long long inc = v;
#pragma unroll
    for (int d = 1; d < 32; d <<= 1) {
        const unsigned long long o = __shfl_up_sync(0xffffffffu, inc, d);
        if (lane >= d) inc += o;
    }
    if (lane == 31) sm[warp] = inc;
    __syncthreads();
    if (warp == 0) {
        const unsigned long long w = sm[lane];
        unsigned long long winc = w;
#pragma unroll
        for (int d = 1; d < 32; d <<= 1) {
            const unsigned long long o = __shfl_up_sync(0xffffffffu, winc, d);
            if (lane >= d) winc += o;
        }
        sm[lane] = winc - w;
        if (lane == 31) sm[32] = winc;
    }
    __syncthreads();
    const unsigned long long ex = sm[warp] + inc - v;
    total = sm[32];
    __syncthreads();
    return ex;
}

__global__ void __launch_bounds__(1024) positions_kernel(const __grid_constant__ EntropyBuffers b, const __grid_constant__ DevPlan P, unsigned long long n_chunks,
                                                         unsigned long long n_segs, int scan_chunks) {
    __shared__ unsigned long long sm[33];
    unsigned long long carry = 0, total;
    if (scan_chunks) {
        for (unsigned long long base = 0; base < n_chunks; base += 1024) {
            const unsigned long long i = base + threadIdx.x;
            const unsigned long long ex = cta1024_exclusive(i < n_chunks ? b.chunk_bits[i] : 0ull, sm, total);
            if (i < n_chunks) b.chunk_bitpos[i] = carry + ex;
            carry += total;
        }
        if (threadIdx.x == 0) b.chunk_bitpos[n_chunks] = carry;
        __syncthreads();
    }
    carry = 0;
    for (unsigned long long base = 0; base < n_segs; base += 1024) {
        const unsigned long long g = base + threadIdx.x;
        unsigned long long bytes = 0;
        if (g < n_segs) {
            bytes = segment_bytes(b, P, g);
            if (bytes > 0xFFFFFFFFull) atomicOr(b.status + 2, 8ull);
        }
        const unsigned long long ex = cta1024_exclusive(bytes, sm, total);
        if (g < n_segs) b.segpos[g] = carry + ex;
        carry += total;
    }
    if (threadIdx.x == 0) b.segpos[n_segs] = carry;
}

__device__ __forceinline__ unsigned long long stream_bytes(const EntropyBuffers &b) { return b.segpos[b.n_segs_total]; }
__device__ __forceinline__ bool stream_fits(const EntropyBuffers &b) { return stream_bytes(b) <= b.ustream_cap; }

__device__ __forceinline__ void put_raw(const EntropyBuffers &b, unsigned long long pos, uint8_t byte) {
    b.ustream[pos] = byte;
    atomicOr(b.raw_mask + (pos >> 5), 1u << (pos & 31));
}

__global__ void __launch_bounds__(128) segment_lead_kernel(const __grid_constant__ EntropyBuffers b, const __grid_constant__ DevPlan P, unsigned long long n_segs,
                                                           const unsigned wps) {
    const unsigned long long gw = ((unsigned long long)blockIdx.x * blockDim.x + threadIdx.x) >> 5;
    const unsigned long long g = gw / wps;
    const unsigned slice = (unsigned)(gw - g * wps);
    const int lane = threadIdx.x & 31;
    if (blockIdx.x == 0 && threadIdx.x == 0) {
        const unsigned long long bytes = stream_bytes(b);
        b.status[0] = bytes;
        if (bytes > b.ustream_cap) atomicOr(b.status + 2, 1ull);
    }
    if (g >= n_segs || !stream_fits(b)) return;
    const unsigned long long img = g / P.segs_per_image;
    const unsigned s = (unsigned)(g - img * P.segs_per_image);
    const int k = find_scan_by_seg(P, s);
    const DevScan &S = P.scans[k];
    const unsigned i = s - S.seg_base;
    const unsigned long long pos = b.segpos[g];
    {
        const bool eoi = s == P.segs_per_image - 1 && P.has_eoi;
        const unsigned cps = P.groups[k % P.n_groups].cps;
        const unsigned long long c0 = img * P.chunks_per_image + S.chunk_base + (unsigned long long)i * cps;
        const unsigned long long bit0 = b.chunk_bitpos[c0];
        const unsigned long long data0 = pos + lead_len(b, P, img, k, i), data1 = b.segpos[g + 1] - (eoi ? 2u : 0u);
        const unsigned per = (cps + wps) / wps;
        const unsigned q1 = (slice + 1) * per < cps + 1 ? (slice + 1) * per : cps + 1;
        for (unsigned q = slice * per + lane; q < q1; q += 32) {
            const unsigned long long pbit = data0 * 8 + (b.chunk_bitpos[c0 + q] - bit0);
            if ((pbit & 31) == 0) continue;
            const unsigned long long w = pbit >> 5;
            const unsigned long long lo = w * 4 > data0 ? w * 4 : data0, hi = w * 4 + 4 < data1 ? w * 4 + 4 : data1;
            if (lo + 4 == hi) reinterpret_cast<uint32_t *>(b.ustream)[w] = 0u;
            else
                for (unsigned long long x = lo; x < hi; ++x) b.ustream[x] = 0;
        }
    }
    if (slice != 0) return;
    if (S.rst_base + i > 0) {
        if (lane == 0) {
            put_raw(b, pos, 0xFF);
            put_raw(b, pos + 1, (uint8_t)(0xD0 + ((S.rst_base + i - 1) & 7)));
        }
    } else if (k > 0) {
        for (unsigned j = lane; j < S.sos_len; j += 32) put_raw(b, pos + j, P.blob[S.sos_off + j]);
    } else {
        const unsigned long long h = b.huff_per_image ? img : 0;
        const unsigned n = b.hdr_len[h];
        const uint8_t *src = b.hdr + h * b.hdr_stride;
#pragma unroll 4
        for (unsigned j = lane; j < n; j += 32) b.ustream[pos + j] = src[j];
        const unsigned long long w0 = pos >> 5, w1 = (pos + n - 1) >> 5;
        for (unsigned long long w = w0 + lane; w <= w1 && n; w += 32) {
            const unsigned long long lo = w * 32 > pos ? w * 32 : pos, hi = (w + 1) * 32 < pos + n ? (w + 1) * 32 : pos + n;
            const unsigned bits = (unsigned)(hi - lo);
            atomicOr(b.raw_mask + w, (bits == 32 ? 0xFFFFFFFFu : ((1u << bits) - 1u)) << (unsigned)(lo & 31));
        }
    }
    if (s == P.segs_per_image - 1 && P.has_eoi && lane == 0) {
        const unsigned long long end = b.segpos[g + 1];
        put_raw(b, end - 2, 0xFF);
        put_raw(b, end - 1, 0xD9);
    }
}

__global__ void __launch_bounds__(256) place_chunks_kernel(const __grid_constant__ EntropyBuffers b, const __grid_constant__ DevPlan P, unsigned long long n_chunks,
                                                           const unsigned per_warp) {
    if (!stream_fits(b) || (b.status[2] & 4ull)) return;
    const int lane = threadIdx.x & 31;
    const unsigned long long warps = ((unsigned long long)gridDim.x * blockDim.x) >> 5;
    uint32_t *stream = reinterpret_cast<uint32_t *>(b.ustream);
    for (unsigned long long c0 = (((unsigned long long)blockIdx.x * blockDim.x + threadIdx.x) >> 5) * per_warp; c0 < n_chunks; c0 += warps * per_warp) {
        const unsigned long long c = c0 + lane;
        unsigned my_bits = 0, my_pool = 0;
        unsigned long long my_bitpos = 0;
        if ((unsigned)lane < per_warp && c < n_chunks) {
            const unsigned long long img = c / P.chunks_per_image;
            const unsigned r = (unsigned)(c - img * P.chunks_per_image);
            const int k = find_scan_by_chunk(P, r);
            const DevScan &S = P.scans[k];
            const DevGroup &G = P.groups[k % P.n_groups];
            unsigned seg, q;
            divmod(r - S.chunk_base, G.div_cps, seg, q);
            my_bits = b.chunk_bits[c];
            if (my_bits != 0 || q == 0) {
                const unsigned long long seg_first = b.chunk_bitpos[c - q];
                const unsigned long long data_byte = b.segpos[img * P.segs_per_image + S.seg_base + seg] + lead_len(b, P, img, k, seg);
                my_bitpos = data_byte * 8 + (b.chunk_bitpos[c] - seg_first);
                if (my_bits) my_pool = b.chunk_pool[c];
                if (q == 0) {
                    const unsigned long long seg_bits = b.chunk_bitpos[c + G.cps] - seg_first;
                    const unsigned pad = (unsigned)(-(long long)seg_bits) & 7u;
                    if (pad) {
                        const unsigned long long pbit = data_byte * 8 + seg_bits;
                        const unsigned s2 = (unsigned)(pbit & 31);
                        atomicOr(stream + (pbit >> 5), __byte_perm(((1u << pad) - 1u) << (32 - s2 - pad), 0, 0x0123));
                    }
                }
            }
        }
        unsigned todo = __ballot_sync(0xffffffffu, my_bits != 0);
        while (todo) {
            const int who = __ffs(todo) - 1;
            todo &= todo - 1;
            const unsigned bits = __shfl_sync(0xffffffffu, my_bits, who);
            const unsigned long long bitpos = __shfl_sync(0xffffffffu, my_bitpos, who);
            const uint32_t *src = b.pool + (size_t)__shfl_sync(0xffffffffu, my_pool, who) * 4;
            const unsigned sft = (unsigned)(bitpos & 31);
            uint32_t *dst = stream + (bitpos >> 5);
            const unsigned nw = (bits + 31) >> 5, ndw = (sft + bits + 31) >> 5;
            const bool first_owned = sft == 0, last_owned = ((sft + bits) & 31) == 0;
            uint32_t carry = 0;
            for (unsigned base = 0; base < ndw; base += 128) {
                uint32_t cur[4];
#pragma unroll
                for (int u = 0; u < 4; ++u) {
                    const unsigned d = base + 32 * u + lane;
                    cur[u] = d < nw ? __ldg(src + d) : 0u;
                }
#pragma unroll
                for (int u = 0; u < 4; ++u) {
                    const unsigned d = base + 32 * u + lane;
                    uint32_t prev = __shfl_up_sync(0xffffffffu, cur[u], 1);
                    if (lane == 0) prev = carry;
                    carry = __shfl_sync(0xffffffffu, cur[u], 31);
                    if (d < ndw) {
                        const uint32_t val = sft ? __funnelshift_r(cur[u], prev, sft) : cur[u];
                        const uint32_t be = __byte_perm(val, 0, 0x0123);
                        const bool owned = (d > 0 || first_owned) && (d + 1 < ndw || last_owned);
                        if (owned) dst[d] = be;
                        else atomicOr(dst + d, be);
                    }
                }
            }
        }
    }
}

__device__ __forceinline__ uint32_t ff_flags(uint32_t w) {
    const uint32_t x = ~w;
    const uint32_t t = ((x & 0x7F7F7F7Fu) + 0x7F7F7F7Fu) | x;
    return ~t & 0x80808080u;
}
__device__ __forceinline__ unsigned flags_to_nibble(uint32_t z) { return (((z >> 7) * 0x00204081u) >> 21) & 0xFu; }

__device__ __forceinline__ unsigned ff_bits16(const uint4 d, unsigned raw16, unsigned valid) {
    unsigned m = flags_to_nibble(ff_flags(d.x)) | flags_to_nibble(ff_flags(d.y)) << 4 | flags_to_nibble(ff_flags(d.z)) << 8 |
                 flags_to_nibble(ff_flags(d.w)) << 12;
    m &= ~raw16;
    if (valid < 16) m &= (1u << valid) - 1u;
    return m;
}
__device__ __forceinline__ unsigned ff_count16(const uint4 d, unsigned raw16, unsigned valid) {
    if (raw16 == 0 && valid >= 16) return __popc(ff_flags(d.x)) + __popc(ff_flags(d.y)) + __popc(ff_flags(d.z)) + __popc(ff_flags(d.w));
    return __popc(ff_bits16(d, raw16, valid));
}

__global__ void __launch_bounds__(256) count_ff_kernel(const EntropyBuffers b) {
    __shared__ unsigned warp_sums[8];
    const unsigned long long bytes = stream_fits(b) ? stream_bytes(b) : 0ull;
    const unsigned long long base = (unsigned long long)blockIdx.x * kStuffChunk + (unsigned long long)threadIdx.x * 16;
    unsigned cnt = 0;
    if (base < bytes) {
        const uint4 d = *reinterpret_cast<const uint4 *>(b.ustream + base);
        const unsigned raw = (b.raw_mask[base >> 5] >> (base & 31)) & 0xFFFFu;
        const unsigned valid = bytes - base < 16 ? (unsigned)(bytes - base) : 16u;
        cnt = ff_count16(d, raw, valid);
    }
    cnt = __reduce_add_sync(0xffffffffu, cnt);
    if ((threadIdx.x & 31) == 0) warp_sums[threadIdx.x >> 5] = cnt;
    __syncthreads();
    if (threadIdx.x == 0) {
        unsigned t = 0;
        for (int i = 0; i < 8; ++i) t += warp_sums[i];
        b.ffcount[blockIdx.x] = t;
    }
}

constexpr unsigned kDirectPieces = 2048;

__device__ __forceinline__ void ff_sums_warp(const uint32_t *ffcount, unsigned n_pieces, unsigned idx, int lane, unsigned long long &before, unsigned long long &total) {
    unsigned a = 0, t = 0;
    for (unsigned j = lane; j < n_pieces; j += 32) {
        const unsigned v = ffcount[j];
        t += v;
        if (j < idx) a += v;
    }
    before = __reduce_add_sync(0xffffffffu, a);
    total = __reduce_add_sync(0xffffffffu, t);
}

__device__ __forceinline__ unsigned ff_before_in_chunk(const EntropyBuffers &b, unsigned long long pos, int lane) {
    const unsigned long long start = pos / kStuffChunk * kStuffChunk;
    unsigned ff = 0;
    for (unsigned long long i = start + (unsigned long long)lane * 16; i < pos; i += 32 * 16) {
        const uint4 d = *reinterpret_cast<const uint4 *>(b.ustream + i);
        const unsigned raw = (b.raw_mask[i >> 5] >> (i & 31)) & 0xFFFFu;
        const unsigned valid = pos - i < 16 ? (unsigned)(pos - i) : 16u;
        ff += ff_count16(d, raw, valid);
    }
    return __reduce_add_sync(0xffffffffu, ff);
}

__global__ void __launch_bounds__(256) stuff_scatter_kernel(const __grid_constant__ EntropyBuffers b, const __grid_constant__ DevPlan P, unsigned n_pieces,
                                                            unsigned n_images, unsigned long long *piece_offs) {
    if (!stream_fits(b)) return;
    const unsigned long long bytes = stream_bytes(b);
    const bool direct = n_pieces <= kDirectPieces;
    const int lane = threadIdx.x & 31, warp = threadIdx.x >> 5;
    if (blockIdx.x >= n_pieces) {
        const unsigned k = (blockIdx.x - n_pieces) * 8 + warp;
        const unsigned n_pos = n_images + 1 + (piece_offs ? (unsigned)P.n_scans + 1 : 0u);
        if (k >= n_pos) return;
        unsigned long long pos;
        unsigned long long *dst;
        if (k <= n_images) {
            pos = k == n_images ? bytes : b.segpos[(unsigned long long)k * P.segs_per_image];
            dst = b.file_off + k;
        } else {
            const unsigned sc = k - (n_images + 1);
            pos = sc == (unsigned)P.n_scans ? bytes : b.segpos[P.scans[sc].seg_base];
            dst = piece_offs + sc;
        }
        const unsigned long long piece = pos / kStuffChunk;
        unsigned long long before, total;
        if (direct) ff_sums_warp(b.ffcount, n_pieces, (unsigned)piece, lane, before, total);
        else before = b.ffpos[piece];
        const unsigned ff = ff_before_in_chunk(b, pos, lane);
        if (lane == 0) *dst = pos + before + ff;
        return;
    }
    __shared__ unsigned warp_excl[9];
    __shared__ unsigned long long ff_sm[2];
    __shared__ __align__(16) uint8_t stage[2 * kStuffChunk + 32];
    unsigned long long ff_before, ff_total;
    if (direct) {
        if (warp == 0) {
            unsigned long long a, t;
            ff_sums_warp(b.ffcount, n_pieces, blockIdx.x, lane, a, t);
            if (lane == 0) ff_sm[0] = a, ff_sm[1] = t;
        }
        __syncthreads();
        ff_before = ff_sm[0];
        ff_total = ff_sm[1];
    } else {
        ff_before = b.ffpos[blockIdx.x];
        ff_total = b.ffpos[n_pieces];
    }
    if (blockIdx.x == 0 && threadIdx.x == 0) {
        b.status[1] = ff_total;
        if (bytes + ff_total > b.out_cap) atomicOr(b.status + 2, 2ull);
    }
    if (bytes + ff_total > b.out_cap) return;
    if ((unsigned long long)blockIdx.x * kStuffChunk >= bytes) return;
    const unsigned long long base = (unsigned long long)blockIdx.x * kStuffChunk + (unsigned long long)threadIdx.x * 16;
    uint4 d = make_uint4(0, 0, 0, 0);
    unsigned m = 0, valid = 0;
    if (base < bytes) {
        d = *reinterpret_cast<const uint4 *>(b.ustream + base);
        const unsigned raw = (b.raw_mask[base >> 5] >> (base & 31)) & 0xFFFFu;
        valid = bytes - base < 16 ? (unsigned)(bytes - base) : 16u;
        m = ff_bits16(d, raw, valid);
    }
    const unsigned cnt = __popc(m);
    unsigned inc = cnt;
#pragma unroll
    for (int o = 1; o < 32; o <<= 1) {
        const unsigned t = __shfl_up_sync(0xffffffffu, inc, o);
        if (lane >= o) inc += t;
    }
    if (lane == 31) warp_excl[warp + 1] = inc;
    __syncthreads();
    if (threadIdx.x == 0) {
        warp_excl[0] = 0;
        for (int i = 1; i <= 8; ++i) warp_excl[i] += warp_excl[i - 1];
    }
    __syncthreads();
    const unsigned long long chunk_base = (unsigned long long)blockIdx.x * kStuffChunk;
    const unsigned long long out0 = chunk_base + ff_before;
    const unsigned pad = (unsigned)(out0 & 15);
    const unsigned chunk_in = bytes - chunk_base < kStuffChunk ? (unsigned)(bytes - chunk_base) : (unsigned)kStuffChunk;
    const unsigned total = chunk_in + warp_excl[8];
    if (valid) {
        unsigned o = pad + threadIdx.x * 16 + warp_excl[warp] + (inc - cnt);
        const uint32_t w[4] = {d.x, d.y, d.z, d.w};
#pragma unroll
        for (int i = 0; i < 16; ++i) {
            if ((unsigned)i < valid) {
                stage[o++] = (uint8_t)(w[i >> 2] >> ((i & 3) * 8));
                if (m & (1u << i)) stage[o++] = 0x00;
            }
        }
    }
    __syncthreads();
    uint8_t *dst = b.out + (out0 - pad);
    const unsigned end = pad + total;
    for (unsigned o = threadIdx.x * 16; o < end; o += 256 * 16) {
        if (o >= pad && o + 16 <= end) {
            *reinterpret_cast<uint4 *>(dst + o) = *reinterpret_cast<const uint4 *>(stage + o);
        } else {
            for (unsigned k = (o < pad ? pad : o); k < o + 16 && k < end; ++k) dst[k] = stage[k];
        }
    }
}

template <int BASE>
__device__ __forceinline__ void count_half(unsigned m, int &next, unsigned c_shared, unsigned *ha) {
#pragma unroll 1
    while (m) {
        int p;
        asm("bfind.u32 %0, %1;" : "=r"(p) : "r"(m));
        unsigned bit;
        asm("bmsk.clamp.b32 %0, %1, 1;" : "=r"(bit) : "r"(p));
        m ^= bit;
        const int k = BASE + 31 - p;
        int v;
        asm("ld.shared.s16 %0, [%1];" : "=r"(v) : "r"(c_shared + 2 * k));
        const int run = k - next;
        next = k + 1;
        const int a = v < 0 ? -v : v;
        int top;
        asm("bfind.u32 %0, %1;" : "=r"(top) : "r"(a));
        atomicAdd(ha + ((run << 4) | (top + 1)), 1u);
    }
}

__global__ void __launch_bounds__(256) histogram_kernel(const __grid_constant__ DevPlan P, const int16_t *coef, unsigned n_images, uint32_t *hist,
                                                        int bands, int per_band) {
    __shared__ unsigned sh[2 * 2 * 257];
    __shared__ __align__(16) int16_t blk[256 * kStageStride];
    const int tid = threadIdx.x;
    const unsigned long long g0 = (unsigned long long)blockIdx.x * 256;
    const unsigned n_here = P.blocks_per_image - g0 < 256 ? (unsigned)(P.blocks_per_image - g0) : 256u;
    for (unsigned img = blockIdx.y; img < n_images; img += gridDim.y) {
        for (int i = tid; i < 2 * 2 * 257; i += 256) sh[i] = 0;
        const int16_t *src = coef + ((unsigned long long)img * P.blocks_per_image + g0) * 64;
        {
            const unsigned pieces = n_here * 8;
            const char *g = reinterpret_cast<const char *>(src) + (size_t)tid * 16;
            const unsigned d = (unsigned)__cvta_generic_to_shared(blk) + (tid >> 3) * (kStageStride * 2) + (tid & 7) * 16;
#pragma unroll
            for (int k = 0; k < 8; ++k)
                if ((unsigned)(tid + k * 256) < pieces)
                    asm volatile("cp.async.cg.shared.global [%0], [%1], 16;" ::"r"(d + k * 32 * (kStageStride * 2)), "l"(g + k * 256 * 16) : "memory");
            asm volatile("cp.async.wait_all;" ::: "memory");
        }
        __syncthreads();
        if ((unsigned)tid < n_here) {
            const unsigned long long g = g0 + tid;
            int comp = 0;
            while (comp + 1 < P.n_groups && g >= P.groups[comp + 1].block_base) ++comp;
            const int16_t *mine = blk + tid * kStageStride;
            const uint4 *m4 = reinterpret_cast<const uint4 *>(mine);
            unsigned m_lo = 0, m_hi = 0;
#pragma unroll
            for (int w = 0; w < 8; ++w) {
                const uint4 q = m4[w];
                unsigned byte = __dp2a_lo(nonzero16x2(q.x), 0x0201u, 0u);
                byte = __dp2a_lo(nonzero16x2(q.y), 0x0804u, byte);
                byte = __dp2a_lo(nonzero16x2(q.z), 0x2010u, byte);
                byte = __dp2a_lo(nonzero16x2(q.w), 0x8040u, byte);
                if (w < 4) m_lo |= byte << (8 * w);
                else m_hi |= byte << (8 * (w - 4));
            }
            const unsigned long long m_all = (((unsigned long long)m_hi << 32) | m_lo) & ~1ull;
            const int prev = g > P.groups[comp].block_base ? (tid > 0 ? (int)mine[-kStageStride] : (int)__ldg(src - 64)) : 0;
            unsigned *h = sh + P.comp_tbl[comp] * 2 * 257;
            const int diff = (int)(int16_t)(mine[0] - prev);
            atomicAdd(h + (32 - __clz(diff < 0 ? -diff : diff)), 1u);
            unsigned *ha = h + 257;
            const unsigned c_shared = (unsigned)__cvta_generic_to_shared(mine);
            for (int b = 0; b < bands; ++b) {
                const int first_ac = b == 0 ? 1 : b * per_band, se = b == bands - 1 ? 63 : (b + 1) * per_band - 1;
                if (se < first_ac) continue;
                unsigned long long m = m_all & (~0ull << first_ac) & (~0ull >> (63 - se));
                m |= zrl_markers(m, first_ac);
                int next = first_ac;
                count_half<0>(__brev((unsigned)m), next, c_shared, ha);
                count_half<32>(__brev((unsigned)(m >> 32)), next, c_shared, ha);
                if (next <= se) atomicAdd(ha, 1u);
            }
        }
        __syncthreads();
        uint32_t *dst = hist + (size_t)img * (2 * 2 * 257);
        for (int i = tid; i < 2 * 2 * 257; i += 256)
            if (sh[i]) atomicAdd(dst + i, sh[i]);
        __syncthreads();
    }
}

}

static inline unsigned grid_for(unsigned long long n, unsigned block) { return (unsigned)((n + block - 1) / block); }

cudaError_t launch_histogram(const DevPlan &hp, const int16_t *coef, uint32_t n_images, uint32_t *hist,
                             cudaStream_t stream) {
    const int bands = hp.spg > 1 ? hp.spg - 1 : 1;
    const int per_band = bands > 1 ? 64 / bands : 64;
    dim3 grid(grid_for(hp.blocks_per_image, 256), n_images < 32768 ? n_images : 32768);
    histogram_kernel<<<grid, 256, 0, stream>>>(hp, coef, n_images, hist, bands, per_band);
    return cudaGetLastError();
}

namespace {
constexpr int kMaxDevices = 64;
struct CoderInfo {
    bool ready = false;
    int n_sms = 0, ctas_per_sm = 0;
};
template <int T, bool FULL>
cudaError_t coder_info(CoderInfo &out) {
    static std::mutex mu;
    static CoderInfo cache[kMaxDevices];
    int dev = 0;
    cudaGetDevice(&dev);
    std::lock_guard<std::mutex> lock(mu);
    CoderInfo &c = cache[dev < kMaxDevices ? dev : kMaxDevices - 1];
    if (!c.ready) {
        auto kernel = encode_chunks_kernel<T, FULL>;
        const int smem = CoderSmem<T, FULL>::kBytes;
        cudaError_t e = cudaFuncSetAttribute(kernel, cudaFuncAttributeMaxDynamicSharedMemorySize, smem);
        if (e != cudaSuccess) return e;
        cudaDeviceGetAttribute(&c.n_sms, cudaDevAttrMultiProcessorCount, dev);
        e = cudaOccupancyMaxActiveBlocksPerMultiprocessor(&c.ctas_per_sm, kernel, T, smem);
        if (e != cudaSuccess) return e;
        if (c.ctas_per_sm < 1) c.ctas_per_sm = 1;
        c.ready = true;
    }
    out = c;
    return cudaSuccess;
}
template <int T, bool FULL>
cudaError_t coder_config(unsigned long long n_items, CoderLaunch &cfg) {
    CoderInfo info;
    cudaError_t e = coder_info<T, FULL>(info);
    if (e != cudaSuccess) return e;
    unsigned long long grid = (unsigned long long)info.n_sms * info.ctas_per_sm;
    if (grid > n_items) grid = n_items;
    if (grid < 1) grid = 1;
    cfg.grid = (unsigned)grid;
    cfg.smem = CoderSmem<T, FULL>::kBytes;
    cfg.scratch_bytes = (size_t)grid * T * kSlotWords * 4;
    return cudaSuccess;
}
inline bool plan_is_full(const DevPlan &hp) { return hp.scans[hp.n_scans - 1].ss == 0 && hp.scans[hp.n_scans - 1].se == 63; }
}

#define JPGB_CODER_DISPATCH(CALL)                              \
    do {                                                       \
        const bool full = plan_is_full(hp);                    \
        switch (hp.chunk_T) {                                  \
        case 32: if (full) { CALL(32, true); } else { CALL(32, false); } break;    \
        case 64: if (full) { CALL(64, true); } else { CALL(64, false); } break;    \
        case 128: if (full) { CALL(128, true); } else { CALL(128, false); } break; \
        default: if (full) { CALL(256, true); } else { CALL(256, false); } break;  \
        }                                                      \
    } while (0)

cudaError_t coder_launch_config(const DevPlan &hp, uint32_t n, CoderLaunch &cfg) {
    const unsigned long long n_items = (unsigned long long)hp.items_per_image * n;
#define JPGB_CFG(T, F) return coder_config<T, F>(n_items, cfg)
    JPGB_CODER_DISPATCH(JPGB_CFG);
#undef JPGB_CFG
    return cudaErrorInvalidValue;
}
cudaError_t launch_encode_chunks(const EntropyBuffers &b, const DevPlan &hp, uint32_t n, const CoderLaunch &cfg, cudaStream_t s) {
    const unsigned long long n_items = (unsigned long long)hp.items_per_image * n;
#define JPGB_RUN(T, F) encode_chunks_kernel<T, F><<<cfg.grid, T, cfg.smem, s>>>(b, hp, n_items)
    JPGB_CODER_DISPATCH(JPGB_RUN);
#undef JPGB_RUN
    return cudaGetLastError();
}
cudaError_t launch_segment_lengths(const EntropyBuffers &b, const DevPlan &hp, uint32_t n, cudaStream_t s) {
    const unsigned long long ns = (unsigned long long)hp.segs_per_image * n;
    segment_len_kernel<<<grid_for(ns, 256), 256, 0, s>>>(b, hp, ns);
    return cudaGetLastError();
}
cudaError_t launch_positions(const EntropyBuffers &b, const DevPlan &hp, uint32_t n, bool scan_chunks, cudaStream_t s) {
    positions_kernel<<<1, 1024, 0, s>>>(b, hp, (unsigned long long)hp.chunks_per_image * n, (unsigned long long)hp.segs_per_image * n, scan_chunks ? 1 : 0);
    return cudaGetLastError();
}
cudaError_t launch_segment_leads(const EntropyBuffers &b, const DevPlan &hp, uint32_t n, cudaStream_t s) {
    const unsigned long long ns = (unsigned long long)hp.segs_per_image * n;
    unsigned cps = 1;
    for (int g = 0; g < hp.n_groups; ++g) cps = hp.groups[g].cps > cps ? hp.groups[g].cps : cps;
    unsigned wps = (cps + 1 + 127) / 128;
    wps = wps > 1024 ? 1024 : wps;
    segment_lead_kernel<<<grid_for(ns * wps * 32, 128), 128, 0, s>>>(b, hp, ns, wps);
    return cudaGetLastError();
}
cudaError_t launch_place_chunks(const EntropyBuffers &b, const DevPlan &hp, uint32_t n, cudaStream_t s) {
    const unsigned long long nc = (unsigned long long)hp.chunks_per_image * n;
    unsigned per_warp = 1;
    while (per_warp < 32 && nc / (per_warp * 2) >= 16384) per_warp *= 2;
    const unsigned long long ctas = (nc + 8ull * per_warp - 1) / (8ull * per_warp);
    place_chunks_kernel<<<(unsigned)(ctas < 65536 ? (ctas ? ctas : 1) : 65536), 256, 0, s>>>(b, hp, nc, per_warp);
    return cudaGetLastError();
}
cudaError_t launch_count_ff(const EntropyBuffers &b, cudaStream_t s) {
    count_ff_kernel<<<grid_for(b.ustream_cap, kStuffChunk), 256, 0, s>>>(b);
    return cudaGetLastError();
}
bool ff_scan_needed(const EntropyBuffers &b) { return grid_for(b.ustream_cap, kStuffChunk) > kDirectPieces; }
cudaError_t launch_stuff_scatter(const EntropyBuffers &b, const DevPlan &hp, uint32_t n, unsigned long long *piece_offs, cudaStream_t s) {
    const unsigned n_pieces = grid_for(b.ustream_cap, kStuffChunk);
    const unsigned n_pos = n + 1 + (piece_offs ? (unsigned)hp.n_scans + 1 : 0u);
    stuff_scatter_kernel<<<n_pieces + (n_pos + 7) / 8, 256, 0, s>>>(b, hp, n_pieces, n, piece_offs);
    return cudaGetLastError();
}

}
```

jpeg_encoder_b200/csrc/kernels.h:

```cpp
#pragma once
#include <cuda_runtime.h>

#include <cstdint>

#include "../../include/jpegenc_b200.h"
#include "device_types.h"

namespace jpgb {

cudaError_t launch_stage_a(const StageAParams &p, uint32_t n_images, cudaStream_t stream);

constexpr size_t kHuffWordsPerImage = 2 * 2 * 256;

struct EntropyBuffers {
    const int16_t *coef;
    const uint32_t *huff;
    int huff_per_image;
    uint32_t *scratch;
    uint32_t *pool;
    unsigned long long pool_cap;
    uint32_t *chunk_bits;
    uint32_t *chunk_pool;
    unsigned long long *chunk_bitpos;
    uint32_t *seglen;
    unsigned long long *segpos;
    const uint32_t *hdr_len;
    const uint8_t *hdr;
    uint32_t hdr_stride;
    uint8_t *ustream;
    uint32_t *raw_mask;
    uint32_t *ffcount;
    unsigned long long *ffpos;
    uint8_t *out;
    unsigned long long *file_off;
    void *scan_tmp;
    unsigned long long ustream_cap, out_cap, n_segs_total;
    unsigned long long *status;
    size_t scan_tmp_bytes;
};
constexpr int kStatusWords = 8;

constexpr int kSlotWords = 56;
constexpr int kStuffChunk = 4096;

cudaError_t launch_histogram(const DevPlan &hplan, const int16_t *coef, uint32_t n_images,
                             uint32_t *hist , cudaStream_t stream);
struct CoderLaunch {
    unsigned grid;
    size_t smem, scratch_bytes;
};
cudaError_t coder_launch_config(const DevPlan &hplan, uint32_t n_images, CoderLaunch &cfg);
cudaError_t launch_encode_chunks(const EntropyBuffers &b, const DevPlan &hplan, uint32_t n_images, const CoderLaunch &cfg, cudaStream_t stream);
cudaError_t launch_segment_lengths(const EntropyBuffers &b, const DevPlan &hplan, uint32_t n_images, cudaStream_t stream);
cudaError_t launch_positions(const EntropyBuffers &b, const DevPlan &hplan, uint32_t n_images, bool scan_chunks, cudaStream_t stream);
cudaError_t launch_segment_leads(const EntropyBuffers &b, const DevPlan &hplan, uint32_t n_images, cudaStream_t stream);
cudaError_t launch_place_chunks(const EntropyBuffers &b, const DevPlan &hplan, uint32_t n_images, cudaStream_t stream);
cudaError_t launch_count_ff(const EntropyBuffers &b, cudaStream_t stream);
bool ff_scan_needed(const EntropyBuffers &b);
cudaError_t launch_stuff_scatter(const EntropyBuffers &b, const DevPlan &hplan, uint32_t n_images, unsigned long long *piece_offs, cudaStream_t stream);

cudaError_t launch_build_tables(const uint32_t *hist, int hist_per_image, int n_tables, uint32_t n_images, uint32_t *huff, const uint8_t *head,
                                uint32_t head_len, const uint8_t *tail, uint32_t tail_len, uint8_t *hdr, uint32_t hdr_stride, uint32_t *hdr_len,
                                unsigned long long *status, cudaStream_t stream);

cudaError_t launch_build_single_tables(const uint32_t *hist, uint32_t n, int ac, uint32_t *words, uint8_t *dht, uint32_t *dht_len, uint32_t *bad,
                                       cudaStream_t stream);

cudaError_t launch_place_pieces(const uint8_t *src, uint8_t *dst, unsigned long long dst_cap, const unsigned long long *table, unsigned world,
                                unsigned rank, unsigned n_scans, unsigned long long *total_out, unsigned long long *status, cudaStream_t stream);

size_t scan_tmp_bytes(uint64_t n);
cudaError_t launch_exclusive_scan(const uint32_t *in, unsigned long long *out, uint64_t n, void *tmp, cudaStream_t stream,
                                  uint32_t *launches, unsigned long long *err_flag = nullptr);

}
```

Before: 309,800.

## Assemble stuffed stream directly from chunk pool via per-piece chunk map

Drops the intermediate unstuffed byte stream and its raw-byte mask. A new piece-map kernel records, for each 4 KiB piece, the first chunk that overlaps it plus a small header of chunk positions. The count-ff and scatter kernels then rebuild the stream bytes on the fly from the pool, with markers and headers located by binary search over segment positions. This removes a full write and a full read of the stream plus the mask atomics. In exchange, bytes are gathered twice (once for counting, once for scattering), each piece needs extra chunk lookups, and segment start offsets are now found by binary search inside the scatter.

```diff
diff --git a/jpeg_encoder_b200/csrc/api.cu b/jpeg_encoder_b200/csrc/api.cu
--- a/jpeg_encoder_b200/csrc/api.cu
+++ b/jpeg_encoder_b200/csrc/api.cu
@@ -129,7 +129,7 @@
     cudaStream_t stream = nullptr;
     bool own_stream = false;
     std::string err;
-    DevBuf pixels, coef, huff, hdr, hdr_len, scratch, pool, chunk_bits, chunk_pool, chunk_bitpos, seglen, segpos, ustream, ffcount, ffpos,
+    DevBuf pixels, coef, huff, hdr, hdr_len, scratch, pool, chunk_bits, chunk_pool, chunk_bitpos, chunk_bit0, seglen, segpos, piece_first, piece_head, ffcount, ffpos,
         out, scan_tmp, hist, piece_off, out2, pixels2, status, aux_status, hdr_parts;
     std::vector<uint8_t> last_tables;
     double ucap_ratio = 0;
@@ -348,6 +348,7 @@
     CK(enc->chunk_bits.reserve(n_chunks * 4), "alloc chunk sizes");
     CK(enc->chunk_pool.reserve(n_chunks * 4), "alloc chunk places");
     CK(enc->chunk_bitpos.reserve((n_chunks + 1) * 8), "alloc chunk positions");
+    CK(enc->chunk_bit0.reserve(n_chunks * 8), "alloc chunk stream positions");
     CK(enc->seglen.reserve(n_segs * 4), "alloc seglen");
     CK(enc->segpos.reserve((n_segs + 1) * 8), "alloc segpos");
     CoderLaunch coder{};
@@ -362,6 +363,7 @@
     b.chunk_bits = enc->chunk_bits.as<uint32_t>();
     b.chunk_pool = enc->chunk_pool.as<uint32_t>();
     b.chunk_bitpos = enc->chunk_bitpos.as<unsigned long long>();
+    b.chunk_bit0 = enc->chunk_bit0.as<unsigned long long>();
     b.seglen = enc->seglen.as<uint32_t>();
     b.segpos = enc->segpos.as<unsigned long long>();
     b.hdr_len = enc->hdr_len.as<uint32_t>();
@@ -399,9 +401,9 @@
     for (int attempt = 0;; ++attempt) {
         ucap = (ucap + kStuffChunk - 1) / kStuffChunk * kStuffChunk;
         const uint64_t n_pieces = ucap / kStuffChunk;
-        CK(enc->ustream.reserve(ucap + 64), "alloc unstuffed stream");
-        const size_t mask_bytes = (size_t)(ucap / 32 + 2) * 4;
-        CK(enc->status.reserve((size_t)(n + 1 + 2 * kStatusWords) * 8 + mask_bytes), "alloc status and raw mask");
+        CK(enc->piece_first.reserve((n_pieces + 1) * 8), "alloc piece map");
+        CK(enc->piece_head.reserve((n_pieces + 1) * sizeof(PieceHead)), "alloc piece heads");
+        CK(enc->status.reserve((size_t)(n + 1 + 2 * kStatusWords) * 8), "alloc status");
         CK(enc->ffcount.reserve((n_pieces + 1) * 4), "alloc ff counts");
         CK(enc->ffpos.reserve((n_pieces + 2) * 8), "alloc ff positions");
         CK(enc->scan_tmp.reserve(scan_tmp_bytes(std::max<uint64_t>(n_pieces, std::max(n_chunks, n_segs)))), "alloc scan scratch");
@@ -414,12 +416,12 @@
         }
         b.pool = enc->pool.as<uint32_t>();
         b.pool_cap = pool_units;
-        b.ustream = enc->ustream.as<uint8_t>();
+        b.piece_first = enc->piece_first.as<unsigned long long>();
+        b.piece_head = enc->piece_head.as<PieceHead>();
         b.file_off = enc->status.as<unsigned long long>();
         b.status = b.file_off + (n + 1);
         aux_status = b.status + kStatusWords;
         scan_err = b.status + 3;
-        b.raw_mask = reinterpret_cast<uint32_t *>(b.status + 2 * kStatusWords);
         b.ffcount = enc->ffcount.as<uint32_t>();
         b.ffpos = enc->ffpos.as<unsigned long long>();
         b.scan_tmp = enc->scan_tmp.p;
@@ -428,12 +430,7 @@
         b.out_cap = ocap;
         const bool with_tables = optimized && attempt == 0, with_coder = !coded;
         auto enqueue = [&]() -> int {
-            if (with_coder) {
-                CK(cudaMemsetAsync(b.status, 0, 2 * kStatusWords * 8 + mask_bytes, st), "clear status and raw mask");
-            } else {
-                CK(cudaMemsetAsync(b.status, 0, 4 * 8, st), "clear status");
-                CK(cudaMemsetAsync(b.raw_mask, 0, mask_bytes, st), "clear raw mask");
-            }
+            CK(cudaMemsetAsync(b.status, 0, (with_coder ? 2 * kStatusWords : 4) * 8, st), "clear status");
             if (with_tables) {
                 const int rc = enqueue_tables();
                 if (rc != JPGB_OK) return rc;
@@ -456,17 +453,16 @@
             }
             {
                 StageTimer t(enc, 3);
-                if (poison) CK(cudaMemsetAsync(b.ustream, 0xFF, ucap + 64, st), "poison stream");
-                CK(launch_segment_leads(b, hp, n, st), "segment lead launch");
-                CK(launch_place_chunks(b, hp, n, st), "placement launch");
+                if (poison) CK(cudaMemsetAsync(b.out, 0xFF, ocap + 64, st), "poison output");
+                CK(launch_piece_map(b, hp, n, st), "piece map launch");
+                CK(launch_count_ff(b, hp, n, st), "count ff launch");
                 enc->launches += 2;
             }
             {
                 StageTimer t(enc, 4);
-                CK(launch_count_ff(b, st), "count ff launch");
                 if (ff_scan_needed(b)) CK(launch_exclusive_scan(b.ffcount, b.ffpos, n_pieces, b.scan_tmp, st, &enc->launches, scan_err), "ff scan");
                 CK(launch_stuff_scatter(b, hp, n, piece_offsets ? enc->piece_off.as<unsigned long long>() : nullptr, st), "scatter launch");
-                enc->launches += 2;
+                enc->launches += 1;
                 if (piece_offsets)
                     CK(cudaMemcpyAsync(enc->h_pieces.p, enc->piece_off.p, (plan.scans.size() + 1) * 8, cudaMemcpyDeviceToHost, st), "read piece offsets");
                 CK(cudaMemcpyAsync(enc->h_small.p, b.file_off, (size_t)(n + 1 + 2 * kStatusWords) * 8, cudaMemcpyDeviceToHost, st), "read file offsets and status");
@@ -807,8 +803,8 @@
     if (!e) return;
     cudaSetDevice(e->device);
     cudaStreamSynchronize(e->stream);
-    DevBuf *bufs[] = {&e->pixels, &e->coef, &e->huff, &e->hdr, &e->hdr_len, &e->scratch, &e->pool, &e->chunk_bits, &e->chunk_pool, &e->chunk_bitpos, &e->seglen, &e->segpos,
-                      &e->ustream, &e->ffcount, &e->ffpos, &e->out, &e->scan_tmp, &e->hist, &e->piece_off, &e->out2, &e->pixels2, &e->status, &e->aux_status, &e->hdr_parts};
+    DevBuf *bufs[] = {&e->pixels, &e->coef, &e->huff, &e->hdr, &e->hdr_len, &e->scratch, &e->pool, &e->chunk_bits, &e->chunk_pool, &e->chunk_bitpos, &e->chunk_bit0, &e->seglen, &e->segpos,
+                      &e->piece_first, &e->piece_head, &e->ffcount, &e->ffpos, &e->out, &e->scan_tmp, &e->hist, &e->piece_off, &e->out2, &e->pixels2, &e->status, &e->aux_status, &e->hdr_parts};
     for (DevBuf *b : bufs) b->release();
     e->h_small.release();
     e->h_hist.release();
diff --git a/jpeg_encoder_b200/csrc/entropy.cu b/jpeg_encoder_b200/csrc/entropy.cu
--- a/jpeg_encoder_b200/csrc/entropy.cu
+++ b/jpeg_encoder_b200/csrc/entropy.cu
@@ -520,148 +520,83 @@
 }
 
 __device__ __forceinline__ unsigned long long stream_bytes(const EntropyBuffers &b) { return b.segpos[b.n_segs_total]; }
-__device__ __forceinline__ bool stream_fits(const EntropyBuffers &b) { return stream_bytes(b) <= b.ustream_cap; }
-
-__device__ __forceinline__ void put_raw(const EntropyBuffers &b, unsigned long long pos, uint8_t byte) {
-    b.ustream[pos] = byte;
-    atomicOr(b.raw_mask + (pos >> 5), 1u << (pos & 31));
-}
-
-__global__ void __launch_bounds__(128) segment_lead_kernel(const __grid_constant__ EntropyBuffers b, const __grid_constant__ DevPlan P, unsigned long long n_segs,
-                                                           const unsigned wps) {
-    const unsigned long long gw = ((unsigned long long)blockIdx.x * blockDim.x + threadIdx.x) >> 5;
-    const unsigned long long g = gw / wps;
-    const unsigned slice = (unsigned)(gw - g * wps);
-    const int lane = threadIdx.x & 31;
-    if (blockIdx.x == 0 && threadIdx.x == 0) {
-        const unsigned long long bytes = stream_bytes(b);
+__device__ __forceinline__ bool tail_runs(const EntropyBuffers &b) { return stream_bytes(b) <= b.ustream_cap && !(b.status[2] & 4ull); }
+
+__device__ __forceinline__ void chunk_place(const EntropyBuffers &b, const DevPlan &P, unsigned long long c, unsigned long long &bit0,
+                                            unsigned long long &r0, unsigned long long &r1) {
+    const unsigned long long img = c / P.chunks_per_image;
+    const unsigned r = (unsigned)(c - img * P.chunks_per_image);
+    const int k = find_scan_by_chunk(P, r);
+    const DevScan &S = P.scans[k];
+    const DevGroup &G = P.groups[k % P.n_groups];
+    unsigned seg, q;
+    divmod(r - S.chunk_base, G.div_cps, seg, q);
+    const unsigned long long g = img * P.segs_per_image + S.seg_base + seg;
+    const unsigned long long seg_first = b.chunk_bitpos[c - q];
+    const unsigned long long seg0 = b.segpos[g];
+    const unsigned long long data_bit = (seg0 + lead_len(b, P, img, k, seg)) * 8;
+    bit0 = data_bit + (b.chunk_bitpos[c] - seg_first);
+    r0 = q == 0 ? seg0 : (bit0 + 7) >> 3;
+    r1 = q + 1 < G.cps ? (data_bit + (b.chunk_bitpos[c + 1] - seg_first) + 7) >> 3 : b.segpos[g + 1];
+}
+
+__global__ void __launch_bounds__(256) piece_map_kernel(const __grid_constant__ EntropyBuffers b, const __grid_constant__ DevPlan P, unsigned long long n_chunks) {
+    const unsigned long long c = (unsigned long long)blockIdx.x * blockDim.x + threadIdx.x;
+    const unsigned long long bytes = stream_bytes(b);
+    if (c == 0) {
         b.status[0] = bytes;
         if (bytes > b.ustream_cap) atomicOr(b.status + 2, 1ull);
     }
-    if (g >= n_segs || !stream_fits(b)) return;
-    const unsigned long long img = g / P.segs_per_image;
-    const unsigned s = (unsigned)(g - img * P.segs_per_image);
+    if (c >= n_chunks || !tail_runs(b)) return;
+    unsigned long long bit0, r0, r1;
+    chunk_place(b, P, c, bit0, r0, r1);
+    b.chunk_bit0[c] = bit0;
+    unsigned long long p = (r0 + kStuffChunk - 1) / kStuffChunk;
+    if (p * kStuffChunk >= r1) return;
+    PieceHead h;
+    h.bit0[0] = bit0;
+#pragma unroll
+    for (int i = 1; i < kPieceHead; ++i) {
+        unsigned long long x0, x1;
+        h.bit0[i] = 0;
+        if (c + i < n_chunks) chunk_place(b, P, c + i, h.bit0[i], x0, x1);
+    }
+#pragma unroll
+    for (int i = 0; i < kPieceHead; ++i) {
+        h.bits[i] = c + i < n_chunks ? b.chunk_bits[c + i] : 0u;
+        h.pool[i] = c + i < n_chunks ? b.chunk_pool[c + i] : 0u;
+    }
+    for (; p * kStuffChunk < r1; ++p) {
+        b.piece_first[p] = c;
+        b.piece_head[p] = h;
+    }
+}
+
+__device__ __forceinline__ unsigned long long segment_at(const EntropyBuffers &b, unsigned long long x) {
+    unsigned long long lo = 0, hi = b.n_segs_total - 1;
+    while (lo < hi) {
+        const unsigned long long mid = (lo + hi + 1) >> 1;
+        if (b.segpos[mid] <= x) lo = mid;
+        else hi = mid - 1;
+    }
+    return lo;
+}
+
+__device__ __forceinline__ unsigned gap_byte(const EntropyBuffers &b, const DevPlan &P, unsigned long long x) {
+    const unsigned long long lo = segment_at(b, x);
+    const unsigned long long img = lo / P.segs_per_image;
+    const unsigned s = (unsigned)(lo - img * P.segs_per_image);
     const int k = find_scan_by_seg(P, s);
     const DevScan &S = P.scans[k];
     const unsigned i = s - S.seg_base;
-    const unsigned long long pos = b.segpos[g];
-    {
-        const bool eoi = s == P.segs_per_image - 1 && P.has_eoi;
-        const unsigned cps = P.groups[k % P.n_groups].cps;
-        const unsigned long long c0 = img * P.chunks_per_image + S.chunk_base + (unsigned long long)i * cps;
-        const unsigned long long bit0 = b.chunk_bitpos[c0];
-        const unsigned long long data0 = pos + lead_len(b, P, img, k, i), data1 = b.segpos[g + 1] - (eoi ? 2u : 0u);
-        const unsigned per = (cps + wps) / wps;
-        const unsigned q1 = (slice + 1) * per < cps + 1 ? (slice + 1) * per : cps + 1;
-        for (unsigned q = slice * per + lane; q < q1; q += 32) {
-            const unsigned long long pbit = data0 * 8 + (b.chunk_bitpos[c0 + q] - bit0);
-            if ((pbit & 31) == 0) continue;
-            const unsigned long long w = pbit >> 5;
-            const unsigned long long lo = w * 4 > data0 ? w * 4 : data0, hi = w * 4 + 4 < data1 ? w * 4 + 4 : data1;
-            if (lo + 4 == hi) reinterpret_cast<uint32_t *>(b.ustream)[w] = 0u;
-            else
-                for (unsigned long long x = lo; x < hi; ++x) b.ustream[x] = 0;
-        }
-    }
-    if (slice != 0) return;
-    if (S.rst_base + i > 0) {
-        if (lane == 0) {
-            put_raw(b, pos, 0xFF);
-            put_raw(b, pos + 1, (uint8_t)(0xD0 + ((S.rst_base + i - 1) & 7)));
-        }
-    } else if (k > 0) {
-        for (unsigned j = lane; j < S.sos_len; j += 32) put_raw(b, pos + j, P.blob[S.sos_off + j]);
-    } else {
-        const unsigned long long h = b.huff_per_image ? img : 0;
-        const unsigned n = b.hdr_len[h];
-        const uint8_t *src = b.hdr + h * b.hdr_stride;
-#pragma unroll 4
-        for (unsigned j = lane; j < n; j += 32) b.ustream[pos + j] = src[j];
-        const unsigned long long w0 = pos >> 5, w1 = (pos + n - 1) >> 5;
-        for (unsigned long long w = w0 + lane; w <= w1 && n; w += 32) {
-            const unsigned long long lo = w * 32 > pos ? w * 32 : pos, hi = (w + 1) * 32 < pos + n ? (w + 1) * 32 : pos + n;
-            const unsigned bits = (unsigned)(hi - lo);
-            atomicOr(b.raw_mask + w, (bits == 32 ? 0xFFFFFFFFu : ((1u << bits) - 1u)) << (unsigned)(lo & 31));
-        }
-    }
-    if (s == P.segs_per_image - 1 && P.has_eoi && lane == 0) {
-        const unsigned long long end = b.segpos[g + 1];
-        put_raw(b, end - 2, 0xFF);
-        put_raw(b, end - 1, 0xD9);
-    }
-}
-
-__global__ void __launch_bounds__(256) place_chunks_kernel(const __grid_constant__ EntropyBuffers b, const __grid_constant__ DevPlan P, unsigned long long n_chunks,
-                                                           const unsigned per_warp) {
-    if (!stream_fits(b) || (b.status[2] & 4ull)) return;
-    const int lane = threadIdx.x & 31;
-    const unsigned long long warps = ((unsigned long long)gridDim.x * blockDim.x) >> 5;
-    uint32_t *stream = reinterpret_cast<uint32_t *>(b.ustream);
-    for (unsigned long long c0 = (((unsigned long long)blockIdx.x * blockDim.x + threadIdx.x) >> 5) * per_warp; c0 < n_chunks; c0 += warps * per_warp) {
-        const unsigned long long c = c0 + lane;
-        unsigned my_bits = 0, my_pool = 0;
-        unsigned long long my_bitpos = 0;
-        if ((unsigned)lane < per_warp && c < n_chunks) {
-            const unsigned long long img = c / P.chunks_per_image;
-            const unsigned r = (unsigned)(c - img * P.chunks_per_image);
-            const int k = find_scan_by_chunk(P, r);
-            const DevScan &S = P.scans[k];
-            const DevGroup &G = P.groups[k % P.n_groups];
-            unsigned seg, q;
-            divmod(r - S.chunk_base, G.div_cps, seg, q);
-            my_bits = b.chunk_bits[c];
-            if (my_bits != 0 || q == 0) {
-                const unsigned long long seg_first = b.chunk_bitpos[c - q];
-                const unsigned long long data_byte = b.segpos[img * P.segs_per_image + S.seg_base + seg] + lead_len(b, P, img, k, seg);
-                my_bitpos = data_byte * 8 + (b.chunk_bitpos[c] - seg_first);
-                if (my_bits) my_pool = b.chunk_pool[c];
-                if (q == 0) {
-                    const unsigned long long seg_bits = b.chunk_bitpos[c + G.cps] - seg_first;
-                    const unsigned pad = (unsigned)(-(long long)seg_bits) & 7u;
-                    if (pad) {
-                        const unsigned long long pbit = data_byte * 8 + seg_bits;
-                        const unsigned s2 = (unsigned)(pbit & 31);
-                        atomicOr(stream + (pbit >> 5), __byte_perm(((1u << pad) - 1u) << (32 - s2 - pad), 0, 0x0123));
-                    }
-                }
-            }
-        }
-        unsigned todo = __ballot_sync(0xffffffffu, my_bits != 0);
-        while (todo) {
-            const int who = __ffs(todo) - 1;
-            todo &= todo - 1;
-            const unsigned bits = __shfl_sync(0xffffffffu, my_bits, who);
-            const unsigned long long bitpos = __shfl_sync(0xffffffffu, my_bitpos, who);
-            const uint32_t *src = b.pool + (size_t)__shfl_sync(0xffffffffu, my_pool, who) * 4;
-            const unsigned sft = (unsigned)(bitpos & 31);
-            uint32_t *dst = stream + (bitpos >> 5);
-            const unsigned nw = (bits + 31) >> 5, ndw = (sft + bits + 31) >> 5;
-            const bool first_owned = sft == 0, last_owned = ((sft + bits) & 31) == 0;
-            uint32_t carry = 0;
-            for (unsigned base = 0; base < ndw; base += 128) {
-                uint32_t cur[4];
-#pragma unroll
-                for (int u = 0; u < 4; ++u) {
-                    const unsigned d = base + 32 * u + lane;
-                    cur[u] = d < nw ? __ldg(src + d) : 0u;
-                }
-#pragma unroll
-                for (int u = 0; u < 4; ++u) {
-                    const unsigned d = base + 32 * u + lane;
-                    uint32_t prev = __shfl_up_sync(0xffffffffu, cur[u], 1);
-                    if (lane == 0) prev = carry;
-                    carry = __shfl_sync(0xffffffffu, cur[u], 31);
-                    if (d < ndw) {
-                        const uint32_t val = sft ? __funnelshift_r(cur[u], prev, sft) : cur[u];
-                        const uint32_t be = __byte_perm(val, 0, 0x0123);
-                        const bool owned = (d > 0 || first_owned) && (d + 1 < ndw || last_owned);
-                        if (owned) dst[d] = be;
-                        else atomicOr(dst + d, be);
-                    }
-                }
-            }
-        }
-    }
+    const unsigned long long off = x - b.segpos[lo];
+    if (off < lead_len(b, P, img, k, i)) {
+        const unsigned starts = off == 0 && i == 0 ? 0x100u : 0u;
+        if (S.rst_base + i > 0) return off == 0 ? 0xFFu | starts : 0xD0u + ((S.rst_base + i - 1) & 7);
+        if (k > 0) return P.blob[S.sos_off + off] | starts;
+        return b.hdr[(b.huff_per_image ? img : 0) * b.hdr_stride + off] | starts;
+    }
+    return x + 2 == b.segpos[lo + 1] ? 0xFFu : 0xD9u;
 }
 
 __device__ __forceinline__ uint32_t ff_flags(uint32_t w) {
@@ -669,6 +604,7 @@
     const uint32_t t = ((x & 0x7F7F7F7Fu) + 0x7F7F7F7Fu) | x;
     return ~t & 0x80808080u;
 }
+__device__ __forceinline__ uint32_t nonzero_flags(uint32_t w) { return (((w & 0x7F7F7F7Fu) + 0x7F7F7F7Fu) | w) & 0x80808080u; }
 __device__ __forceinline__ unsigned flags_to_nibble(uint32_t z) { return (((z >> 7) * 0x00204081u) >> 21) & 0xFu; }
 
 __device__ __forceinline__ unsigned ff_bits16(const uint4 d, unsigned raw16, unsigned valid) {
@@ -683,16 +619,156 @@
     return __popc(ff_bits16(d, raw16, valid));
 }
 
-__global__ void __launch_bounds__(256) count_ff_kernel(const EntropyBuffers b) {
+__device__ __forceinline__ uint32_t chunk_word(const uint32_t *src, unsigned nw, long long q) {
+    const long long i = q >> 5;
+    const uint32_t hi = (i >= 0 && i < (long long)nw) ? __ldg(src + i) : 0u;
+    const uint32_t lo = (i + 1 >= 0 && i + 1 < (long long)nw) ? __ldg(src + i + 1) : 0u;
+    return __funnelshift_l(lo, hi, (unsigned)(q & 31));
+}
+__device__ __forceinline__ uint32_t bit_range(unsigned lo, unsigned hi) { return (0xFFFFFFFFu >> lo) & ~(hi >= 32 ? 0u : 0xFFFFFFFFu >> hi); }
+
+constexpr int kPieceRecs = 64;
+struct PieceRecs {
+    unsigned long long bit0[kPieceRecs];
+    uint32_t bits[kPieceRecs], pool[kPieceRecs];
+    unsigned long long n;
+    const unsigned long long *bit0_at;
+    const uint32_t *bits_at, *pool_at;
+};
+struct PieceStart {
+    unsigned long long first, next_first, bit0;
+    uint32_t bits, pool;
+};
+__device__ __forceinline__ PieceStart piece_start(const EntropyBuffers &b, unsigned long long p) {
+    PieceStart s;
+    s.first = b.piece_first[p];
+    s.next_first = b.piece_first[p + 1];
+    if (threadIdx.x < kPieceHead) {
+        s.bit0 = b.piece_head[p].bit0[threadIdx.x];
+        s.bits = b.piece_head[p].bits[threadIdx.x];
+        s.pool = b.piece_head[p].pool[threadIdx.x];
+    }
+    return s;
+}
+__device__ __forceinline__ void load_piece_recs(const EntropyBuffers &b, unsigned long long p, unsigned long long bytes, unsigned long long n_chunks,
+                                                const PieceStart &s, PieceRecs &R) {
+    const unsigned long long first = s.first, last = (p + 1) * kStuffChunk < bytes ? s.next_first : n_chunks - 1;
+    const unsigned long long n = last - first + 1;
+    if (n <= kPieceHead) {
+        if (threadIdx.x < n) {
+            R.bit0[threadIdx.x] = s.bit0;
+            R.bits[threadIdx.x] = s.bits;
+            R.pool[threadIdx.x] = s.pool;
+        }
+        if (threadIdx.x == 0) R.bit0_at = R.bit0, R.bits_at = R.bits, R.pool_at = R.pool;
+    } else if (n <= kPieceRecs) {
+        if (threadIdx.x < n) {
+            R.bit0[threadIdx.x] = b.chunk_bit0[first + threadIdx.x];
+            R.bits[threadIdx.x] = b.chunk_bits[first + threadIdx.x];
+            R.pool[threadIdx.x] = b.chunk_pool[first + threadIdx.x];
+        }
+        if (threadIdx.x == 0) R.bit0_at = R.bit0, R.bits_at = R.bits, R.pool_at = R.pool;
+    } else if (threadIdx.x == 0) {
+        R.bit0_at = b.chunk_bit0 + first, R.bits_at = b.chunk_bits + first, R.pool_at = b.chunk_pool + first;
+    }
+    if (threadIdx.x == 0) R.n = n;
+    __syncthreads();
+}
+
+__device__ __forceinline__ uint4 stream_bytes16(const EntropyBuffers &b, const DevPlan &P, const PieceRecs &R, unsigned long long x,
+                                                unsigned long long bytes, unsigned &raw16, unsigned &starts16, unsigned &valid) {
+    valid = bytes - x < 16 ? (unsigned)(bytes - x) : 16u;
+    const unsigned long long X = x * 8, n = R.n;
+    const unsigned long long *bit0_at = R.bit0_at;
+    unsigned long long j = 0;
+    {
+        unsigned long long hi = n - 1;
+        while (j < hi) {
+            const unsigned long long mid = (j + hi + 1) >> 1;
+            if (bit0_at[mid] <= X) j = mid;
+            else hi = mid - 1;
+        }
+    }
+    uint32_t w[4] = {0u, 0u, 0u, 0u}, cov[4] = {0u, 0u, 0u, 0u};
+    bool full = false;
+    for (; j < n; ++j) {
+        const unsigned long long bit0 = bit0_at[j];
+        if (bit0 >= X + 128) break;
+        const unsigned nbits = R.bits_at[j];
+        const unsigned long long e = bit0 + nbits;
+        if (e <= X) continue;
+        const uint32_t *src = b.pool + (size_t)R.pool_at[j] * 4;
+        const long long o = (long long)(X - bit0);
+        if (o >= 0 && e >= X + 128) {
+            const unsigned i = (unsigned)(o >> 5), s = (unsigned)(o & 31), k = i & 3;
+            const uint4 *src4 = reinterpret_cast<const uint4 *>(src) + (i >> 2);
+            const uint4 u = __ldg(src4), v = (k || s) ? __ldg(src4 + 1) : make_uint4(0, 0, 0, 0);
+            const uint32_t a0 = k == 0 ? u.x : k == 1 ? u.y : k == 2 ? u.z : u.w;
+            const uint32_t a1 = k == 0 ? u.y : k == 1 ? u.z : k == 2 ? u.w : v.x;
+            const uint32_t a2 = k == 0 ? u.z : k == 1 ? u.w : k == 2 ? v.x : v.y;
+            const uint32_t a3 = k == 0 ? u.w : k == 1 ? v.x : k == 2 ? v.y : v.z;
+            const uint32_t a4 = k == 0 ? v.x : k == 1 ? v.y : k == 2 ? v.z : v.w;
+            w[0] = __funnelshift_l(a1, a0, s);
+            w[1] = __funnelshift_l(a2, a1, s);
+            w[2] = __funnelshift_l(a3, a2, s);
+            w[3] = __funnelshift_l(a4, a3, s);
+            full = true;
+            break;
+        }
+        const unsigned nw = (nbits + 31) >> 5;
+        const unsigned a = bit0 > X ? (unsigned)(bit0 - X) : 0u, z = e - X < 128 ? (unsigned)(e - X) : 128u;
+#pragma unroll
+        for (int t = 0; t < 4; ++t) {
+            const unsigned lo = a > 32u * t ? a : 32u * t, hi = z < 32u * t + 32 ? z : 32u * t + 32;
+            if (lo < hi) {
+                const uint32_t m = bit_range(lo - 32 * t, hi - 32 * t);
+                w[t] |= chunk_word(src, nw, o + 32 * t) & m;
+                cov[t] |= m;
+            }
+        }
+    }
+    raw16 = 0;
+    starts16 = 0;
+    uint4 d;
+    if (full) {
+        d = make_uint4(__byte_perm(w[0], 0, 0x0123), __byte_perm(w[1], 0, 0x0123), __byte_perm(w[2], 0, 0x0123), __byte_perm(w[3], 0, 0x0123));
+    } else {
+        uint32_t v[4];
+#pragma unroll
+        for (int t = 0; t < 4; ++t) {
+            const uint32_t c = __byte_perm(cov[t], 0, 0x0123), f = nonzero_flags(c);
+            v[t] = __byte_perm(w[t], 0, 0x0123) | (((f >> 7) * 0xFFu) & ~c);
+            raw16 |= flags_to_nibble(~f & 0x80808080u) << (4 * t);
+        }
+        if (valid < 16) raw16 &= (1u << valid) - 1u;
+        for (unsigned todo = raw16; todo; todo &= todo - 1) {
+            const int i = __ffs(todo) - 1;
+            const unsigned g = gap_byte(b, P, x + i), byte = (g & 0xFFu) << ((i & 3) * 8), t = i >> 2;
+            v[0] |= t == 0 ? byte : 0u;
+            v[1] |= t == 1 ? byte : 0u;
+            v[2] |= t == 2 ? byte : 0u;
+            v[3] |= t == 3 ? byte : 0u;
+            if (g & 0x100u) starts16 |= 1u << i;
+        }
+        d = make_uint4(v[0], v[1], v[2], v[3]);
+    }
+    return d;
+}
+
+__global__ void __launch_bounds__(256) count_ff_kernel(const __grid_constant__ EntropyBuffers b, const __grid_constant__ DevPlan P, unsigned long long n_chunks) {
     __shared__ unsigned warp_sums[8];
-    const unsigned long long bytes = stream_fits(b) ? stream_bytes(b) : 0ull;
+    __shared__ PieceRecs recs;
+    const PieceStart start = piece_start(b, blockIdx.x);
+    const unsigned long long bytes = tail_runs(b) ? stream_bytes(b) : 0ull;
     const unsigned long long base = (unsigned long long)blockIdx.x * kStuffChunk + (unsigned long long)threadIdx.x * 16;
     unsigned cnt = 0;
-    if (base < bytes) {
-        const uint4 d = *reinterpret_cast<const uint4 *>(b.ustream + base);
-        const unsigned raw = (b.raw_mask[base >> 5] >> (base & 31)) & 0xFFFFu;
-        const unsigned valid = bytes - base < 16 ? (unsigned)(bytes - base) : 16u;
-        cnt = ff_count16(d, raw, valid);
+    if ((unsigned long long)blockIdx.x * kStuffChunk < bytes) {
+        load_piece_recs(b, blockIdx.x, bytes, n_chunks, start, recs);
+        if (base < bytes) {
+            unsigned raw, starts, valid;
+            const uint4 d = stream_bytes16(b, P, recs, base, bytes, raw, starts, valid);
+            cnt = ff_count16(d, raw, valid);
+        }
     }
     cnt = __reduce_add_sync(0xffffffffu, cnt);
     if ((threadIdx.x & 31) == 0) warp_sums[threadIdx.x >> 5] = cnt;
@@ -717,50 +793,19 @@
     total = __reduce_add_sync(0xffffffffu, t);
 }
 
-__device__ __forceinline__ unsigned ff_before_in_chunk(const EntropyBuffers &b, unsigned long long pos, int lane) {
-    const unsigned long long start = pos / kStuffChunk * kStuffChunk;
-    unsigned ff = 0;
-    for (unsigned long long i = start + (unsigned long long)lane * 16; i < pos; i += 32 * 16) {
-        const uint4 d = *reinterpret_cast<const uint4 *>(b.ustream + i);
-        const unsigned raw = (b.raw_mask[i >> 5] >> (i & 31)) & 0xFFFFu;
-        const unsigned valid = pos - i < 16 ? (unsigned)(pos - i) : 16u;
-        ff += ff_count16(d, raw, valid);
-    }
-    return __reduce_add_sync(0xffffffffu, ff);
-}
-
 __global__ void __launch_bounds__(256) stuff_scatter_kernel(const __grid_constant__ EntropyBuffers b, const __grid_constant__ DevPlan P, unsigned n_pieces,
-                                                            unsigned n_images, unsigned long long *piece_offs) {
-    if (!stream_fits(b)) return;
+                                                            unsigned n_images, unsigned long long n_chunks, unsigned long long *piece_offs) {
+    const bool direct = n_pieces <= kDirectPieces;
+    const PieceStart start = piece_start(b, blockIdx.x);
+    unsigned long long ff_before = direct ? 0ull : b.ffpos[blockIdx.x], ff_total = direct ? 0ull : b.ffpos[n_pieces];
+    if (!tail_runs(b)) return;
     const unsigned long long bytes = stream_bytes(b);
-    const bool direct = n_pieces <= kDirectPieces;
     const int lane = threadIdx.x & 31, warp = threadIdx.x >> 5;
-    if (blockIdx.x >= n_pieces) {
-        const unsigned k = (blockIdx.x - n_pieces) * 8 + warp;
-        const unsigned n_pos = n_images + 1 + (piece_offs ? (unsigned)P.n_scans + 1 : 0u);
-        if (k >= n_pos) return;
-        unsigned long long pos;
-        unsigned long long *dst;
-        if (k <= n_images) {
-            pos = k == n_images ? bytes : b.segpos[(unsigned long long)k * P.segs_per_image];
-            dst = b.file_off + k;
-        } else {
-            const unsigned sc = k - (n_images + 1);
-            pos = sc == (unsigned)P.n_scans ? bytes : b.segpos[P.scans[sc].seg_base];
-            dst = piece_offs + sc;
-        }
-        const unsigned long long piece = pos / kStuffChunk;
-        unsigned long long before, total;
-        if (direct) ff_sums_warp(b.ffcount, n_pieces, (unsigned)piece, lane, before, total);
-        else before = b.ffpos[piece];
-        const unsigned ff = ff_before_in_chunk(b, pos, lane);
-        if (lane == 0) *dst = pos + before + ff;
-        return;
-    }
     __shared__ unsigned warp_excl[9];
     __shared__ unsigned long long ff_sm[2];
+    __shared__ PieceRecs recs;
     __shared__ __align__(16) uint8_t stage[2 * kStuffChunk + 32];
-    unsigned long long ff_before, ff_total;
+    for (unsigned i = threadIdx.x; i < (2 * kStuffChunk + 32) / 16; i += 256) reinterpret_cast<uint4 *>(stage)[i] = make_uint4(0, 0, 0, 0);
     if (direct) {
         if (warp == 0) {
             unsigned long long a, t;
@@ -770,23 +815,22 @@
         __syncthreads();
         ff_before = ff_sm[0];
         ff_total = ff_sm[1];
-    } else {
-        ff_before = b.ffpos[blockIdx.x];
-        ff_total = b.ffpos[n_pieces];
     }
     if (blockIdx.x == 0 && threadIdx.x == 0) {
         b.status[1] = ff_total;
         if (bytes + ff_total > b.out_cap) atomicOr(b.status + 2, 2ull);
+        b.file_off[n_images] = bytes + ff_total;
+        if (piece_offs) piece_offs[P.n_scans] = bytes + ff_total;
     }
     if (bytes + ff_total > b.out_cap) return;
     if ((unsigned long long)blockIdx.x * kStuffChunk >= bytes) return;
+    load_piece_recs(b, blockIdx.x, bytes, n_chunks, start, recs);
     const unsigned long long base = (unsigned long long)blockIdx.x * kStuffChunk + (unsigned long long)threadIdx.x * 16;
     uint4 d = make_uint4(0, 0, 0, 0);
-    unsigned m = 0, valid = 0;
+    unsigned m = 0, valid = 0, starts = 0;
     if (base < bytes) {
-        d = *reinterpret_cast<const uint4 *>(b.ustream + base);
-        const unsigned raw = (b.raw_mask[base >> 5] >> (base & 31)) & 0xFFFFu;
-        valid = bytes - base < 16 ? (unsigned)(bytes - base) : 16u;
+        unsigned raw;
+        d = stream_bytes16(b, P, recs, base, bytes, raw, starts, valid);
         m = ff_bits16(d, raw, valid);
     }
     const unsigned cnt = __popc(m);
@@ -808,25 +852,56 @@
     const unsigned pad = (unsigned)(out0 & 15);
     const unsigned chunk_in = bytes - chunk_base < kStuffChunk ? (unsigned)(bytes - chunk_base) : (unsigned)kStuffChunk;
     const unsigned total = chunk_in + warp_excl[8];
-    if (valid) {
-        unsigned o = pad + threadIdx.x * 16 + warp_excl[warp] + (inc - cnt);
-        const uint32_t w[4] = {d.x, d.y, d.z, d.w};
+    uint32_t *stage32 = reinterpret_cast<uint32_t *>(stage);
+    const unsigned o = pad + threadIdx.x * 16 + warp_excl[warp] + (inc - cnt);
+    if (valid == 16 && m == 0) {
+        const unsigned s = (o & 3) * 8, w0 = o >> 2;
+        atomicOr(stage32 + w0, __funnelshift_l(0u, d.x, s));
+        stage32[w0 + 1] = __funnelshift_l(d.x, d.y, s);
+        stage32[w0 + 2] = __funnelshift_l(d.y, d.z, s);
+        stage32[w0 + 3] = __funnelshift_l(d.z, d.w, s);
+        if (s) atomicOr(stage32 + w0 + 4, __funnelshift_l(d.w, 0u, s));
+    } else if (valid) {
+        const uint32_t in[4] = {d.x, d.y, d.z, d.w};
+        unsigned at = o;
+        uint32_t acc = 0;
+        auto put = [&](uint32_t byte) {
+            acc |= byte << ((at & 3) * 8);
+            ++at;
+            if ((at & 3) == 0) {
+                const unsigned wi = (at >> 2) - 1;
+                if (wi == (o >> 2)) atomicOr(stage32 + wi, acc);
+                else stage32[wi] = acc;
+                acc = 0;
+            }
+        };
 #pragma unroll
         for (int i = 0; i < 16; ++i) {
             if ((unsigned)i < valid) {
-                stage[o++] = (uint8_t)(w[i >> 2] >> ((i & 3) * 8));
-                if (m & (1u << i)) stage[o++] = 0x00;
-            }
-        }
+                put((in[i >> 2] >> ((i & 3) * 8)) & 0xFFu);
+                if (m & (1u << i)) put(0u);
+            }
+        }
+        if (at & 3) atomicOr(stage32 + (at >> 2), acc);
+    }
+    for (unsigned todo = starts; todo; todo &= todo - 1) {
+        const int i = __ffs(todo) - 1;
+        const unsigned long long x = base + i;
+        const unsigned long long at = out0 + (o - pad) + i + __popc(m & ((1u << i) - 1u));
+        const unsigned long long seg = segment_at(b, x);
+        const unsigned long long img = seg / P.segs_per_image;
+        const unsigned s = (unsigned)(seg - img * P.segs_per_image);
+        if (s == 0) b.file_off[img] = at;
+        if (piece_offs && img == 0) piece_offs[find_scan_by_seg(P, s)] = at;
     }
     __syncthreads();
     uint8_t *dst = b.out + (out0 - pad);
     const unsigned end = pad + total;
-    for (unsigned o = threadIdx.x * 16; o < end; o += 256 * 16) {
-        if (o >= pad && o + 16 <= end) {
-            *reinterpret_cast<uint4 *>(dst + o) = *reinterpret_cast<const uint4 *>(stage + o);
+    for (unsigned q = threadIdx.x * 16; q < end; q += 256 * 16) {
+        if (q >= pad && q + 16 <= end) {
+            *reinterpret_cast<uint4 *>(dst + q) = *reinterpret_cast<const uint4 *>(stage + q);
         } else {
-            for (unsigned k = (o < pad ? pad : o); k < o + 16 && k < end; ++k) dst[k] = stage[k];
+            for (unsigned k = (q < pad ? pad : q); k < q + 16 && k < end; ++k) dst[k] = stage[k];
         }
     }
 }
@@ -1007,32 +1082,19 @@
     positions_kernel<<<1, 1024, 0, s>>>(b, hp, (unsigned long long)hp.chunks_per_image * n, (unsigned long long)hp.segs_per_image * n, scan_chunks ? 1 : 0);
     return cudaGetLastError();
 }
-cudaError_t launch_segment_leads(const EntropyBuffers &b, const DevPlan &hp, uint32_t n, cudaStream_t s) {
-    const unsigned long long ns = (unsigned long long)hp.segs_per_image * n;
-    unsigned cps = 1;
-    for (int g = 0; g < hp.n_groups; ++g) cps = hp.groups[g].cps > cps ? hp.groups[g].cps : cps;
-    unsigned wps = (cps + 1 + 127) / 128;
-    wps = wps > 1024 ? 1024 : wps;
-    segment_lead_kernel<<<grid_for(ns * wps * 32, 128), 128, 0, s>>>(b, hp, ns, wps);
+cudaError_t launch_piece_map(const EntropyBuffers &b, const DevPlan &hp, uint32_t n, cudaStream_t s) {
+    const unsigned long long nc = (unsigned long long)hp.chunks_per_image * n;
+    piece_map_kernel<<<grid_for(nc, 256), 256, 0, s>>>(b, hp, nc);
     return cudaGetLastError();
 }
-cudaError_t launch_place_chunks(const EntropyBuffers &b, const DevPlan &hp, uint32_t n, cudaStream_t s) {
-    const unsigned long long nc = (unsigned long long)hp.chunks_per_image * n;
-    unsigned per_warp = 1;
-    while (per_warp < 32 && nc / (per_warp * 2) >= 16384) per_warp *= 2;
-    const unsigned long long ctas = (nc + 8ull * per_warp - 1) / (8ull * per_warp);
-    place_chunks_kernel<<<(unsigned)(ctas < 65536 ? (ctas ? ctas : 1) : 65536), 256, 0, s>>>(b, hp, nc, per_warp);
-    return cudaGetLastError();
-}
-cudaError_t launch_count_ff(const EntropyBuffers &b, cudaStream_t s) {
-    count_ff_kernel<<<grid_for(b.ustream_cap, kStuffChunk), 256, 0, s>>>(b);
+cudaError_t launch_count_ff(const EntropyBuffers &b, const DevPlan &hp, uint32_t n, cudaStream_t s) {
+    count_ff_kernel<<<grid_for(b.ustream_cap, kStuffChunk), 256, 0, s>>>(b, hp, (unsigned long long)hp.chunks_per_image * n);
     return cudaGetLastError();
 }
 bool ff_scan_needed(const EntropyBuffers &b) { return grid_for(b.ustream_cap, kStuffChunk) > kDirectPieces; }
 cudaError_t launch_stuff_scatter(const EntropyBuffers &b, const DevPlan &hp, uint32_t n, unsigned long long *piece_offs, cudaStream_t s) {
     const unsigned n_pieces = grid_for(b.ustream_cap, kStuffChunk);
-    const unsigned n_pos = n + 1 + (piece_offs ? (unsigned)hp.n_scans + 1 : 0u);
-    stuff_scatter_kernel<<<n_pieces + (n_pos + 7) / 8, 256, 0, s>>>(b, hp, n_pieces, n, piece_offs);
+    stuff_scatter_kernel<<<n_pieces, 256, 0, s>>>(b, hp, n_pieces, n, (unsigned long long)hp.chunks_per_image * n, piece_offs);
     return cudaGetLastError();
 }
 
diff --git a/jpeg_encoder_b200/csrc/kernels.h b/jpeg_encoder_b200/csrc/kernels.h
--- a/jpeg_encoder_b200/csrc/kernels.h
+++ b/jpeg_encoder_b200/csrc/kernels.h
@@ -11,6 +11,12 @@
 cudaError_t launch_stage_a(const StageAParams &p, uint32_t n_images, cudaStream_t stream);
 
 constexpr size_t kHuffWordsPerImage = 2 * 2 * 256;
+
+constexpr int kPieceHead = 4;
+struct PieceHead {
+    unsigned long long bit0[kPieceHead];
+    uint32_t bits[kPieceHead], pool[kPieceHead];
+};
 
 struct EntropyBuffers {
     const int16_t *coef;
@@ -27,8 +33,9 @@
     const uint32_t *hdr_len;
     const uint8_t *hdr;
     uint32_t hdr_stride;
-    uint8_t *ustream;
-    uint32_t *raw_mask;
+    unsigned long long *chunk_bit0;
+    unsigned long long *piece_first;
+    PieceHead *piece_head;
     uint32_t *ffcount;
     unsigned long long *ffpos;
     uint8_t *out;
@@ -53,9 +60,8 @@
 cudaError_t launch_encode_chunks(const EntropyBuffers &b, const DevPlan &hplan, uint32_t n_images, const CoderLaunch &cfg, cudaStream_t stream);
 cudaError_t launch_segment_lengths(const EntropyBuffers &b, const DevPlan &hplan, uint32_t n_images, cudaStream_t stream);
 cudaError_t launch_positions(const EntropyBuffers &b, const DevPlan &hplan, uint32_t n_images, bool scan_chunks, cudaStream_t stream);
-cudaError_t launch_segment_leads(const EntropyBuffers &b, const DevPlan &hplan, uint32_t n_images, cudaStream_t stream);
-cudaError_t launch_place_chunks(const EntropyBuffers &b, const DevPlan &hplan, uint32_t n_images, cudaStream_t stream);
-cudaError_t launch_count_ff(const EntropyBuffers &b, cudaStream_t stream);
+cudaError_t launch_piece_map(const EntropyBuffers &b, const DevPlan &hplan, uint32_t n_images, cudaStream_t stream);
+cudaError_t launch_count_ff(const EntropyBuffers &b, const DevPlan &hplan, uint32_t n_images, cudaStream_t stream);
 bool ff_scan_needed(const EntropyBuffers &b);
 cudaError_t launch_stuff_scatter(const EntropyBuffers &b, const DevPlan &hplan, uint32_t n_images, unsigned long long *piece_offs, cudaStream_t stream);
 
```

Result: slower. 252,900, median of 6 (-18.4%).
